# mavmap/mavmap

Hardware: AMD Instinct MI355X
Metric: global-BA LM iterations/sec (higher is better)
Workload: dtype f64; 1 GPU; C3: 500 images / 200000 points / 2000000 obs global BA, PINHOLE+OPENCV, 2 shared cameras; images=500, points=200000, observations=2000000, parallelism=single GPU, options=max_iter 200, ftol 1e-6, gtol 1e-10, ptol 1e-8, Cauchy a=1, refine intrinsics

## Files before the change

__graft_entry__.py:

```python
import os
import subprocess
import sys

ROOT = os.path.dirname(os.path.abspath(__file__))
if ROOT not in sys.path:
    sys.path.insert(0, ROOT)


REFERENCE_FM_SHIM_DEPS = (("tests", "shim", "shim_driver.cpp"), ("tests", "shim", "mock_mavba.cpp"), ("shim", "base3d", "bundle_adjustment.cc"),
                          ("shim", "base3d", "bundle_adjustment.h"), ("include", "mavba.h"))


def build() -> None:
    from mavmap_amd import build as b
    lib = b.build()
    assert os.path.exists(lib), lib
    subprocess.check_call(["make", "-C", os.path.join(ROOT, "oracle"), "-s"])
    subprocess.check_call(["make", "-C", os.path.join(ROOT, "oracle"), "-s", "-B", "ref"])
    ref_shim = os.path.join(ROOT, "oracle", "_ref", "_shim_mock_reffm.so")
    if os.path.exists(ref_shim):
        with open(ref_shim + ".sha256", "w") as fh:
            fh.write(b.files_digest(os.path.join(ROOT, *f) for f in REFERENCE_FM_SHIM_DEPS))
    host_src = os.path.join(ROOT, "tests", "host", "ba_math_host.cpp")
    host_so = os.path.join(ROOT, "tests", "host", "_ba_math_host.so")
    subprocess.check_call(["g++", "-O2", "-std=c++17", "-fPIC", "-shared", "-o", host_so, host_src])
    tri_src = os.path.join(ROOT, "tests", "host", "tri_math_host.cpp")
    tri_so = os.path.join(ROOT, "tests", "host", "_tri_math_host.so")
    subprocess.check_call(["g++", "-O2", "-std=c++17", "-fPIC", "-shared", "-o", tri_so, tri_src])
    p3p_src = os.path.join(ROOT, "tests", "host", "p3p_math_host.cpp")
    p3p_so = os.path.join(ROOT, "tests", "host", "_p3p_math_host.so")
    subprocess.check_call(["g++", "-O2", "-std=c++17", "-fPIC", "-shared", "-o", p3p_so, p3p_src])
    e5_src = os.path.join(ROOT, "tests", "host", "e5_math_host.cpp")
    e5_so = os.path.join(ROOT, "tests", "host", "_e5_math_host.so")
    subprocess.check_call(["g++", "-O2", "-std=c++17", "-fPIC", "-shared", "-o", e5_so, e5_src])
    import mavmap_amd
    L = mavmap_amd.load()
    from mavmap_amd import api
    for sym in api.EXPORTED_SYMBOLS + api.TRIANGULATE_SYMBOLS + api.ABSPOSE_SYMBOLS + api.RELPOSE_SYMBOLS + api.BACKSUB_TILES_SYMBOLS:
        getattr(L, sym)


def smoke() -> None:
    import mavmap_amd
    from mavmap_amd import synth
    from tests import oracle_lib

    if mavmap_amd.device_count() < 1:
        raise RuntimeError("smoke(): no HIP device visible — the mavba backend has no CPU path")
    p = synth.make_config("C3", scale=0.01, seed=7)
    opts = dict(max_num_iterations=200, function_tolerance=1e-6, gradient_tolerance=1e-10)
    pg, po = p.copy(), p.copy()
    cost, res = mavmap_amd.bundle_adjustment(pg, opts)
    oracle_lib.set_threads(1)
    ro, _ = oracle_lib.solve(po, oracle_lib.options(**opts))
    from tests.conftest import param_errors
    rel = abs(res["final_cost"] - ro["final_cost"]) / ro["final_cost"]
    errs = param_errors(pg, po)
    print(f"smoke: {p.num_images} images / {p.num_points} points / {p.num_obs} obs; "
          f"iterations {res['num_successful_steps'] + res['num_unsuccessful_steps']}; RMSE {cost:.6f} px; "
          f"vs oracle: cost {rel:.2e}, " + ", ".join(f"{k} {v:.1e}" for k, v in errs.items()))
    assert res["final_cost"] < res["initial_cost"]
    assert rel < 1e-6 and all(v < 1e-6 for v in errs.values()), (rel, errs)


if __name__ == "__main__":
    build()
    if "--smoke" in sys.argv:
        smoke()
```

mavmap_amd/api.py:

```python
import ctypes as C
import os
from dataclasses import dataclass

import numpy as np

from . import _abi as A
from .problem import BAProblem

_LIB_PATH = os.path.join(os.path.dirname(os.path.abspath(__file__)), "lib", "libmavba.so")
_lib = None

EXPORTED_SYMBOLS = [
    "mavba_options_init", "mavba_last_error", "mavba_device_count", "mavba_solve", "mavba_pose_refine",
    "mavba_session_create", "mavba_session_destroy", "mavba_session_reset", "mavba_session_iterate",
    "mavba_session_result", "mavba_session_get_params", "mavba_session_point_errors",
    "mavba_session_set_allreduce", "mavba_session_eval_jacobian", "mavba_session_reduced_dim",
    "mavba_session_reduced_system", "mavba_session_linear_step", "mavba_session_time_jacobian", "mavba_session_time_front", "mavba_session_set_profiling",
    "mavba_session_kernel_stats", "mavba_session_get_info", "mavba_dense_spd_solve",
    "mavba_scene_create", "mavba_scene_destroy", "mavba_scene_set_camera", "mavba_scene_set_image", "mavba_scene_add_point2d",
    "mavba_scene_add_points2d", "mavba_scene_set_point3d", "mavba_scene_link", "mavba_scene_delete_point3d", "mavba_scene_get_image", "mavba_scene_get_point3d",
    "mavba_scene_get_camera", "mavba_scene_flatten", "mavba_scene_bundle_adjust",
    "mavba_rccl_unique_id", "mavba_session_set_rccl", "mavba_pose_refine_batch", "mavba_session_set_params", "mavba_session_restart", "mavba_session_filter_points", "mavba_solve_filter_solve",
    "mavba_debug_elimination_tree", "mavba_debug_radix_sort", "mavba_debug_lm_decide", "mavba_debug_chol_schedule",
    "mavba_debug_inproc_comms", "mavba_debug_upload_batch",
]
TRIANGULATE_SYMBOLS = ["mavba_triangulate_pairs"]
ABSPOSE_SYMBOLS = ["mavba_absolute_pose_ransac"]
RELPOSE_SYMBOLS = ["mavba_relative_pose_ransac"]
BACKSUB_TILES_SYMBOLS = ["mavba_debug_backsub_tiles"]

ALLREDUCE_FN = C.CFUNCTYPE(C.c_int, C.c_void_p, C.c_void_p, C.c_int64, C.c_int32)


class MavbaError(RuntimeError):
    def __init__(self, code, msg):
        super().__init__(f"mavba error {code}: {msg}")
        self.code = code


def lib_path():
    return _LIB_PATH


def load():
    global _lib
    if _lib is not None:
        return _lib
    if not os.path.exists(_LIB_PATH):
        raise MavbaError(A.ERR_NO_DEVICE, f"{_LIB_PATH} is missing: run `python -m mavmap_amd.build` "
                                          "(the HIP extension is mandatory, there is no CPU fallback)")
    L = C.CDLL(_LIB_PATH)
    dp, ip, bp = C.POINTER(C.c_double), C.POINTER(C.c_int32), C.POINTER(C.c_uint8)
    pp, op, rp = C.POINTER(A.CProblem), C.POINTER(A.COptions), C.POINTER(A.CResult)
    sp = C.c_void_p
    L.mavba_options_init.argtypes = [op]
    L.mavba_options_init.restype = None
    L.mavba_last_error.restype = C.c_char_p
    L.mavba_device_count.restype = C.c_int
    L.mavba_solve.argtypes = [pp, op, rp, dp]
    L.mavba_pose_refine.argtypes = [dp, dp, dp, C.c_int32, dp, dp, bp, C.c_int64, op, rp]
    L.mavba_session_create.argtypes = [pp, op, C.POINTER(sp)]
    L.mavba_session_destroy.argtypes = [sp]
    L.mavba_session_destroy.restype = None
    L.mavba_session_reset.argtypes = [sp]
    L.mavba_session_iterate.argtypes = [sp, C.c_int32, ip, ip]
    L.mavba_session_result.argtypes = [sp, rp]
    L.mavba_session_get_params.argtypes = [sp, dp, dp, dp]
    L.mavba_session_point_errors.argtypes = [sp, dp]
    L.mavba_session_set_allreduce.argtypes = [sp, ALLREDUCE_FN, C.c_void_p, C.c_int32, C.c_int32]
    L.mavba_session_eval_jacobian.argtypes = [sp, dp, dp, dp, dp, dp]
    L.mavba_session_reduced_dim.argtypes = [sp]
    L.mavba_session_reduced_system.argtypes = [sp, C.c_double, dp, dp]
    L.mavba_session_linear_step.argtypes = [sp, C.c_double, dp, dp, dp, dp]
    L.mavba_session_time_jacobian.argtypes = [sp, C.c_int32, C.POINTER(C.c_float)]
    L.mavba_session_time_front.argtypes = [sp, C.c_double, C.c_int32, C.POINTER(C.c_float)]
    L.mavba_session_set_profiling.argtypes = [sp, C.c_int32]
    L.mavba_session_kernel_stats.argtypes = [sp, C.POINTER(A.CKernelStat), C.c_int32]
    L.mavba_session_get_info.argtypes = [sp, C.POINTER(A.CSessionInfo)]
    L.mavba_dense_spd_solve.argtypes = [C.c_int32, dp, dp, dp, C.c_int32]
    i64p, i64 = C.POINTER(C.c_int64), C.c_int64
    sop = C.POINTER(A.CSceneOptions)
    L.mavba_scene_create.argtypes = [C.POINTER(sp)]
    L.mavba_scene_destroy.argtypes = [sp]
    L.mavba_scene_destroy.restype = None
    L.mavba_scene_set_camera.argtypes = [sp, i64, C.c_int32, dp]
    L.mavba_scene_set_image.argtypes = [sp, i64, i64, dp, dp]
    L.mavba_scene_add_point2d.argtypes = [sp, i64, i64, dp]
    L.mavba_scene_add_points2d.argtypes = [sp, i64, i64, i64p, dp, i64p]
    L.mavba_scene_set_point3d.argtypes = [sp, i64, dp]
    L.mavba_scene_link.argtypes = [sp, i64, i64]
    L.mavba_scene_delete_point3d.argtypes = [sp, i64]
    L.mavba_scene_get_image.argtypes = [sp, i64, dp, dp]
    L.mavba_scene_get_point3d.argtypes = [sp, i64, dp]
    L.mavba_scene_get_camera.argtypes = [sp, i64, ip, dp]
    lists = [i64p, i64, i64p, i64, i64p, i64, i64p, i64, i64p, dp, i64]
    L.mavba_scene_flatten.argtypes = [sp] + lists + [sop, pp, C.POINTER(i64p), C.POINTER(i64p), C.POINTER(i64p)]
    L.mavba_scene_bundle_adjust.argtypes = [sp] + lists + [sop, op, rp, dp, C.POINTER(i64p), C.POINTER(dp), i64p]
    L.mavba_rccl_unique_id.argtypes = [C.c_void_p]
    L.mavba_session_set_rccl.argtypes = [sp, C.c_void_p, C.c_int32, C.c_int32]
    L.mavba_pose_refine_batch.argtypes = [C.c_int32, C.POINTER(A.CPoseRefineItem), op, rp]
    L.mavba_triangulate_pairs.argtypes = [C.c_int32, C.POINTER(A.CTriPair), C.c_int32]
    L.mavba_triangulate_pairs.restype = C.c_int
    L.mavba_absolute_pose_ransac.argtypes = [C.c_int32, C.POINTER(A.CAbsPoseItem), C.c_int32]
    L.mavba_absolute_pose_ransac.restype = C.c_int
    L.mavba_relative_pose_ransac.argtypes = [C.c_int32, C.POINTER(A.CRelPoseItem), C.c_int32]
    L.mavba_relative_pose_ransac.restype = C.c_int
    L.mavba_session_set_params.argtypes = [sp, dp, dp, dp]
    L.mavba_session_restart.argtypes = [sp]
    L.mavba_session_filter_points.argtypes = [sp, C.c_double, bp, bp, dp, C.POINTER(C.c_int64)]
    L.mavba_solve_filter_solve.argtypes = [pp, op, C.c_double, bp, rp, rp, dp, bp, C.POINTER(C.c_int64)]
    L.mavba_debug_elimination_tree.argtypes = [C.c_int32, C.c_int32, C.c_int64, ip, ip, C.c_int32, ip, ip, C.c_int32]
    L.mavba_debug_radix_sort.argtypes = [C.c_int32, C.POINTER(C.c_uint32), C.c_int32, ip, C.c_int32]
    L.mavba_debug_lm_decide.argtypes = [C.c_int32, dp, dp, dp, C.c_int32]
    L.mavba_debug_backsub_tiles.argtypes = [C.c_int32, ip, ip, C.c_int32]
    L.mavba_debug_backsub_tiles.restype = C.c_int
    i32p, i64p = C.POINTER(C.c_int32), C.POINTER(C.c_int64)
    L.mavba_debug_chol_schedule.argtypes = [C.c_int32, C.c_int32, i32p, i32p, i32p, C.c_int64, i32p, i32p, C.c_int32, dp,
                                            i32p, C.c_int64, i64p, i32p, C.c_int64, i64p, i32p]
    for f in EXPORTED_SYMBOLS:
        if f not in ("mavba_options_init", "mavba_last_error", "mavba_session_destroy", "mavba_scene_destroy", "mavba_debug_upload_batch"):
            getattr(L, f).restype = C.c_int
    _lib = L
    return L


def _check(rc):
    if rc != A.OK:
        raise MavbaError(rc, load().mavba_last_error().decode(errors="replace"))


def device_count():
    return int(load().mavba_device_count())


def _d(a):
    return A.ptr(a, C.c_double)


@dataclass
class BundleAdjustmentOptions:
    max_num_iterations: int = 100
    function_tolerance: float = 1e-4
    gradient_tolerance: float = 1e-8
    update_point3D_errors: bool = False
    min_track_len: int = 2
    loss_scale_factor: float = 1.0
    constrain_rotation: bool = False
    constrain_rotation_weight: float = 0.0
    refine_camera_params: bool = False
    print_progress: bool = False
    print_summary: bool = True

    @staticmethod
    def global_ba():
# ... 467 lines not shown
        self.close()

    def reset(self):
        _check(load().mavba_session_reset(self._h))

    def iterate(self, max_iters=1):
        done, term = C.c_int32(), C.c_int32()
        _check(load().mavba_session_iterate(self._h, int(max_iters), C.byref(done), C.byref(term)))
        return done.value, term.value

    def solve(self):
        self.iterate(self.copt.max_num_iterations + 1)
        return self.result()

    def result(self):
        r = A.CResult()
        _check(load().mavba_session_result(self._h, C.byref(r)))
        return r.as_dict()

    def get_params(self):
        p = self.problem
        poses, intr, pts = np.zeros((p.num_images, 6)), np.zeros((p.num_cameras, 9)), np.zeros((p.num_points, 3))
        _check(load().mavba_session_get_params(self._h, _d(poses), _d(intr), _d(pts)))
        return poses, intr, pts

    def point_errors(self):
        e = np.full(self.problem.num_points, np.nan)
        _check(load().mavba_session_point_errors(self._h, _d(e)))
        return e

    def set_params(self, poses=None, intrinsics=None, points=None):
        p = self.problem
        arrs = [None if a is None else A.as_f64(a, shape) for a, shape in
                ((poses, (p.num_images, 6)), (intrinsics, (p.num_cameras, 9)), (points, (p.num_points, 3)))]
        _check(load().mavba_session_set_params(self._h, *[None if a is None else _d(a) for a in arrs]))

    def restart(self):
        _check(load().mavba_session_restart(self._h))

    def filter_points(self, max_error, keep=None):
        n = self.problem.num_points
        removed, errors = np.zeros(n, np.uint8), np.full(n, np.nan)
        keep_arr = None if keep is None else np.ascontiguousarray(keep, dtype=np.uint8)
        cnt = C.c_int64()
        _check(load().mavba_session_filter_points(self._h, float(max_error), A.ptr(keep_arr, C.c_uint8),
                                                  A.ptr(removed, C.c_uint8), _d(errors), C.byref(cnt)))
        return removed, errors

    def set_allreduce(self, fn, rank, world_size):
        def trampoline(_ctx, ptr, count, op):
            try:
                fn(ptr, count, op)
                return 0
            except Exception as e:
                print("all-reduce hook raised:", repr(e), flush=True)
                return 1
        self._cb = ALLREDUCE_FN(trampoline)
        _check(load().mavba_session_set_allreduce(self._h, self._cb, None, rank, world_size))

    def set_rccl(self, unique_id, rank, world_size):
        buf = C.create_string_buffer(bytes(unique_id), 128)
        _check(load().mavba_session_set_rccl(self._h, buf, rank, world_size))

    def eval_jacobian(self):
        n = self.problem.num_obs
        r, Jc, Jp, Jk = np.zeros((n, 2)), np.zeros((n, 2, 6)), np.zeros((n, 2, 3)), np.zeros((n, 2, 9))
        cost = C.c_double()
        _check(load().mavba_session_eval_jacobian(self._h, C.byref(cost), _d(r), _d(Jc), _d(Jp), _d(Jk)))
        return cost.value, r, Jc, Jp, Jk

    def reduced_system(self, radius):
        n = load().mavba_session_reduced_dim(self._h)
        S, v = np.zeros((n, n)), np.zeros(n)
        _check(load().mavba_session_reduced_system(self._h, float(radius), _d(S), _d(v)))
        return S, v

    def linear_step(self, radius):
        p = self.problem
        dp, di, dx = np.zeros((p.num_images, 6)), np.zeros((p.num_cameras, 9)), np.zeros((p.num_points, 3))
        mcc = C.c_double()
        _check(load().mavba_session_linear_step(self._h, float(radius), _d(dp), _d(di), _d(dx), C.byref(mcc)))
        return dict(d_poses=dp, d_intr=di, d_points=dx, model_cost_change=mcc.value)

    def set_profiling(self, on):
        _check(load().mavba_session_set_profiling(self._h, 1 if on else 0))

    def time_front(self, radius=1e4, reps=20):
        ms = C.c_float(0)
        _check(load().mavba_session_time_front(self._h, float(radius), int(reps), C.byref(ms)))
        return ms.value

    def time_jacobian(self, reps=20):
        ms = C.c_float()
        _check(load().mavba_session_time_jacobian(self._h, int(reps), C.byref(ms)))
        return float(ms.value)

    def info(self):
        i = A.CSessionInfo()
        _check(load().mavba_session_get_info(self._h, C.byref(i)))
        d = {k: getattr(i, k) for k, _ in i._fields_ if k != "schur_terms"}
        d["schur_terms"] = list(i.schur_terms)
        return d

    def kernel_stats(self):
        buf = (A.CKernelStat * 64)()
        n = load().mavba_session_kernel_stats(self._h, buf, 64)
        return {buf[i].name.decode(): dict(launches=int(buf[i].launches), total_ms=float(buf[i].total_ms))
                for i in range(min(n, 64))}


def elimination_tree(num_images, num_cameras, pairs, max_depth=3):
    pairs = np.ascontiguousarray(pairs, dtype=np.int32).reshape(-1, 2)
    a, b = np.ascontiguousarray(pairs[:, 0]), np.ascontiguousarray(pairs[:, 1])
    node = np.zeros(max(num_images, 1), np.int32)
    parent = np.zeros(4096, np.int32)
    n = load().mavba_debug_elimination_tree(int(num_images), int(num_cameras), len(a), A.ptr(a, C.c_int32), A.ptr(b, C.c_int32),
                                           int(max_depth), A.ptr(node, C.c_int32), A.ptr(parent, C.c_int32), len(parent))
    if n < 0:
        _check(n)
    return node[:num_images], parent[:n]


def backsub_tiles(pt_start):
    pt_start = np.ascontiguousarray(pt_start, dtype=np.int32)
    num_points = max(len(pt_start) - 1, 0)
    out = np.zeros((max(num_points, 1), 4), np.int32)
    n = load().mavba_debug_backsub_tiles(num_points, A.ptr(pt_start, C.c_int32), A.ptr(out, C.c_int32), num_points)
    if n < 0:
        _check(n)
    return out[:n].copy()


def radix_sort_order(keys, key_bytes=4, device=-1):
    keys = np.ascontiguousarray(keys, dtype=np.uint32)
    out = np.zeros(len(keys), np.int32)
    _check(load().mavba_debug_radix_sort(len(keys), A.ptr(keys, C.c_uint32), int(key_bytes), A.ptr(out, C.c_int32), device))
    return out


def debug_upload_batch(sizes, arena_bytes=0, device=-1):
    sizes = np.ascontiguousarray(sizes, dtype=np.int64)
    f = load().mavba_debug_upload_batch
    f.restype = C.c_int64
    r = f(C.c_int32(len(sizes)), A.ptr(sizes, C.c_int64), C.c_int64(int(arena_bytes)), C.c_int32(device))
    if r < 0:
        raise MavbaError(A.ERR_HIP, load().mavba_last_error().decode(errors="replace"))
    return int(r)


def debug_lm_decide(cases, device=-1):
    cases = np.ascontiguousarray(cases, dtype=np.float64)
    n = cases.shape[0]
    assert cases.shape[1] == 24
    oh, od = np.zeros((n, 6)), np.zeros((n, 6))
    _check(load().mavba_debug_lm_decide(n, _d(cases), _d(oh), _d(od), device))
    return oh, od


def debug_chol_schedule(nb, nodes, pairs, cus=256):
    nodes = np.ascontiguousarray(nodes, dtype=np.int32).reshape(-1, 3)
    pairs = np.ascontiguousarray(pairs, dtype=np.int32).reshape(-1, 2)
    nbg, ne, npar = (np.ascontiguousarray(nodes[:, k]) for k in range(3))
    pr, pc = np.ascontiguousarray(pairs[:, 0]), np.ascontiguousarray(pairs[:, 1])
    i32 = lambda a: a.ctypes.data_as(C.POINTER(C.c_int32))
    out = np.zeros(8)
    nt, nu = C.c_int64(), C.c_int64()
# ... 25 lines not shown
```

mavmap_amd/build.py:

```python
import os
import shutil
import subprocess
import sys

ROOT = os.path.dirname(os.path.abspath(__file__))
CSRC = os.path.join(ROOT, "csrc")
LIBDIR = os.path.join(ROOT, "lib")
LIB = os.path.join(LIBDIR, "libmavba.so")
OBJDIR = os.path.join(LIBDIR, "obj")
SOURCES = ["kernels.hip", "schur_rows.hip", "dense_chol.hip", "pose_refine.hip", "triangulate.hip", "absolute_pose.hip", "relative_pose.hip", "host_util.hip", "session_build.hip", "session_lm.hip", "scene.hip", "multi_gpu.hip", "device_setup.hip", "api.hip"]
HEADERS = ["ba_math.h", "tri_math.h", "p3p_math.h", "e5_math.h", "dev_reduce.h", "internal.h", "session.h", "lm_decide.h", "lm_bodies.h", "sweep_body.h", "launch_dispatch.h", os.path.join("..", "..", "include", "mavba.h"),
           os.path.join("..", "..", "include", "mavba_triangulate.h"), os.path.join("..", "..", "include", "mavba_absolute_pose.h"),
           os.path.join("..", "..", "include", "mavba_relative_pose.h"), os.path.join("..", "..", "include", "mavba_backsub_tiles.h")]
FLAGS = ["--offload-arch=gfx950", "-O3", "-std=c++17", "-fPIC", "-ffp-contract=on", "-Wall",
         "-Wno-unused-result"]
FILE_FLAGS = {"dense_chol.hip": ["-mllvm", "-amdgpu-mfma-vgpr-form=1"]}


def _hipcc():
    for cand in (shutil.which("hipcc"), "/opt/rocm/bin/hipcc"):
        if cand and os.path.exists(cand):
            return cand
    raise RuntimeError("hipcc not found (ROCm toolchain required to build libmavba.so)")


STAMP = os.path.join(LIBDIR, "build_stamp.json")


def files_digest(paths):
    import hashlib
    h = hashlib.sha256()
    for p in paths:
        with open(p, "rb") as fh:
            h.update(os.path.basename(p).encode() + b"\0" + fh.read())
    return h.hexdigest()


def source_digest():
    import hashlib
    h = hashlib.sha256()
    for f in SOURCES + HEADERS:
        with open(os.path.normpath(os.path.join(CSRC, f)), "rb") as fh:
            h.update(f.encode() + b"\0" + fh.read())
    h.update(" ".join(FLAGS).encode())
    h.update(repr(sorted(FILE_FLAGS.items())).encode())
    return h.hexdigest()


def is_current():
    import json
    try:
        return os.path.exists(LIB) and json.load(open(STAMP))["digest"] == source_digest()
    except (OSError, ValueError, KeyError):
        return False


def _stale(target, deps):
    if not os.path.exists(target):
        return True
    t = os.path.getmtime(target)
    return any(os.path.getmtime(d) > t for d in deps if os.path.exists(d))


def build(force=False, verbose=False):
    if not force and is_current():
        return LIB
    os.makedirs(OBJDIR, exist_ok=True)
    hdrs = [os.path.normpath(os.path.join(CSRC, h)) for h in HEADERS]
    hipcc = _hipcc()
    objs = []
    for src in SOURCES:
        sp = os.path.join(CSRC, src)
        obj = os.path.join(OBJDIR, src.replace(".hip", ".o"))
        if force or _stale(obj, [sp] + hdrs):
            cmd = [hipcc] + FLAGS + FILE_FLAGS.get(src, []) + ["-c", sp, "-o", obj]
            if verbose:
                print(" ".join(cmd), file=sys.stderr)
            subprocess.check_call(cmd)
        objs.append(obj)
    if force or _stale(LIB, objs):
        cmd = [hipcc, "--offload-arch=gfx950", "-shared", "-fPIC", "-o", LIB] + objs
        if verbose:
            print(" ".join(cmd), file=sys.stderr)
        subprocess.check_call(cmd)
    if not is_current():
        import json
        with open(STAMP, "w") as fh:
            json.dump(dict(digest=source_digest()), fh)
    return LIB


if __name__ == "__main__":
    print(build(force="--force" in sys.argv, verbose=True))
```

mavmap_amd/csrc/api.hip:

```cpp
#include "session.h"
#include "lm_decide.h"

namespace mavba { thread_local std::string g_last_error; }

using namespace mavba;


#define MAVBA_TRY try {
namespace {
struct DeviceGuard {
  int prev = -1;
  explicit DeviceGuard(int dev) {
    if (hipGetDevice(&prev) != hipSuccess) { (void)hipGetLastError(); prev = -1; }
    if (prev != dev) HIP_OK(hipSetDevice(dev)); else prev = -1;
  }
  ~DeviceGuard() { if (prev >= 0) (void)hipSetDevice(prev); }
  DeviceGuard(const DeviceGuard&) = delete;
  DeviceGuard& operator=(const DeviceGuard&) = delete;
};
}
#define MAVBA_SESSION_TRY(s)                                                    \
  try {                                                                         \
    if (!(s)) throw Failure(MAVBA_ERR_INVALID_ARGUMENT, "null session");        \
    DeviceGuard device_guard_((s)->device);
// ... 302 lines not shown

int mavba_debug_backsub_tiles(int32_t NP, const int32_t* pt_start, int32_t* tiles_out, int32_t cap) {
  MAVBA_TRY
  if (NP < 0 || !pt_start || cap < 0 || (cap > 0 && !tiles_out)) throw Failure(MAVBA_ERR_INVALID_ARGUMENT, "bad argument");
  for (int q = 0; q < NP; ++q)
    if (pt_start[q + 1] < pt_start[q]) throw Failure(MAVBA_ERR_BAD_INDEX, "pt_start must not decrease");
  const std::vector<BsTile> tiles = build_backsub_tiles(pt_start, NP);
  if ((long long)tiles.size() > cap) throw Failure(MAVBA_ERR_INVALID_ARGUMENT, "tiles_out too small");
  for (size_t t = 0; t < tiles.size(); ++t) {
    tiles_out[4 * t] = tiles[t].p0; tiles_out[4 * t + 1] = tiles[t].np; tiles_out[4 * t + 2] = tiles[t].o0; tiles_out[4 * t + 3] = tiles[t].no;
  }
  return (int)tiles.size();
  MAVBA_CATCH
}

int mavba_debug_elimination_tree(int32_t NI, int32_t NC, int64_t npairs, const int32_t* pair_a, const int32_t* pair_b, int32_t max_depth,
                                 int32_t* node_of_image, int32_t* node_parent, int32_t cap) {
  MAVBA_TRY
  if (NI < 0 || NC < 0 || npairs < 0 || (npairs > 0 && (!pair_a || !pair_b)) || !node_of_image || !node_parent)
    throw Failure(MAVBA_ERR_INVALID_ARGUMENT, "bad argument");
  std::vector<std::vector<int>> lower(NI);
  for (int64_t k = 0; k < npairs; ++k) {
    const int a = pair_a[k], b = pair_b[k];
    if (a < 0 || a >= NI || b < 0 || b >= NI) throw Failure(MAVBA_ERR_BAD_INDEX, "image pair out of range");
    if (a != b) lower[std::max(a, b)].push_back(std::min(a, b));
  }
  const std::vector<ElimNode> tn = elimination_tree(NI, NC, lower, -1, max_depth);
  if ((int)tn.size() > cap) throw Failure(MAVBA_ERR_INVALID_ARGUMENT, "node_parent too small");
  for (int i = 0; i < NI; ++i) node_of_image[i] = -1;
  for (size_t t = 0; t < tn.size(); ++t) {
    node_parent[t] = tn[t].parent;
    for (int i : tn[t].imgs) node_of_image[i] = (int)t;
  }
  return (int)tn.size();
  MAVBA_CATCH
}

int mavba_session_reduced_system(mavba_session* s, double radius, double* Sout, double* vout) {
  MAVBA_SESSION_TRY(s)
  if (!s->evaluated) s->evaluate();
  s->assemble(radius);
  const int n = s->n_full, m = s->n_mat, nbt = m / 64;
  std::vector<double> store(s->chol_struct.store_doubles());
  s->download(store.data(), s->d_M.p, store.size() * 8);
  s->sync();
  std::vector<double> h((size_t)(m + 1) * m, 0.0);
  const std::vector<int>& slot = s->chol_struct.tile_slot;
  for (int tr = 0; tr <= nbt; ++tr)
    for (int tc = 0; tc < nbt; ++tc) {
      const int sl = slot[(size_t)tr * nbt + tc];
      if (sl < 0) continue;
      const double* T = &store[(size_t)sl << 12];
      const int rows = tr < nbt ? 64 : 1;
      for (int r = 0; r < rows; ++r) std::memcpy(&h[(size_t)(64 * tr + r) * m + 64 * tc], T + 64 * r, 64 * 8);
    }
  std::vector<int> var_col(n, 0);
  for (int t = 0; t < m; ++t) if (s->h_col_var[t] >= 0) var_col[s->h_col_var[t]] = t;
  if (Sout)
    for (int r = 0; r < n; ++r)
      for (int c = 0; c < n; ++c) {
        const int a = std::max(var_col[r], var_col[c]), b = std::min(var_col[r], var_col[c]);
        Sout[(size_t)r * n + c] = h[(size_t)a * m + b];
      }
  if (vout)
    for (int r = 0; r < n; ++r) vout[r] = h[(size_t)m * m + var_col[r]];
  return MAVBA_OK;
  MAVBA_CATCH
}

int mavba_session_linear_step(mavba_session* s, double radius, double* d_poses, double* d_intr, double* d_points,
                              double* model_cost_change) {
  MAVBA_SESSION_TRY(s)
  if (!s->evaluated) s->evaluate();
  double h[SC_COUNT];
  s->linear_step(radius, h);
  if (model_cost_change) *model_cost_change = h[SC_MODEL_CHANGE];
  if (d_poses && s->NI) s->download(d_poses, s->d_delta_cam.p, (size_t)s->NI * 48);
  if (d_intr && s->NC) s->download(d_intr, s->d_delta_cam.p + 6 * (size_t)s->NI, (size_t)s->NC * 72);
  std::vector<double> hdp;
  if (d_points && s->NP) { hdp.resize((size_t)s->NP * 3); s->download(hdp.data(), s->d_delta_pts.p, (size_t)s->NP * 24); }
  s->sync();
  if (d_points) s->to_caller_points(hdp.data(), d_points, 3);
  if (h[SC_FAIL] != 0.0 || h[SC_FAIL_FRONT] != 0.0) throw Failure(MAVBA_ERR_INVALID_ARGUMENT, "linear solve failed (matrix not positive definite)");
  return MAVBA_OK;
  MAVBA_CATCH
}

int mavba_session_time_jacobian(mavba_session* s, int32_t reps, float* ms_avg) {
  MAVBA_SESSION_TRY(s)
  if (reps < 1) reps = 1;
  s->ensure_planes();
  launch_cam_prepare(s->st, s->NI, s->d_poses.p, s->d_camrec.p);
  SweepArgs a = s->sweep_args(s->d_camrec.p, s->d_intr.p, s->d_points.p);
  for (int i = 0; i < 200; ++i) launch_jacobian_sweep(s->st, a);
  std::vector<hipEvent_t> ev((size_t)reps + 1);
  for (auto& e : ev) HIP_OK(hipEventCreate(&e));
  HIP_OK(hipEventRecord(ev[0], s->st));
  for (int i = 0; i < reps; ++i) {
    launch_jacobian_sweep(s->st, a);
    HIP_OK(hipEventRecord(ev[(size_t)i + 1], s->st));
  }
  HIP_OK(hipStreamSynchronize(s->st));
  float ms = 0.f;
  for (int i = 0; i < reps; ++i) {
    float one = 0.f;
    HIP_OK(hipEventElapsedTime(&one, ev[(size_t)i], ev[(size_t)i + 1]));
    ms += one;
  }
  for (auto& e : ev) (void)hipEventDestroy(e);
  if (ms_avg) *ms_avg = ms / reps;
  s->sync();
  return MAVBA_OK;
  MAVBA_CATCH
}

int mavba_debug_chol_schedule(int32_t nb, int32_t num_nodes, const int32_t* node_begin, const int32_t* node_end, const int32_t* node_parent,
                              int64_t num_pairs, const int32_t* pair_row, const int32_t* pair_col, int32_t cus, double* out,
                              int32_t* tasks_out, int64_t tasks_cap, int64_t* num_tasks, int32_t* upd_out, int64_t upd_cap,
                              int64_t* num_upd, int32_t* chain_info_out) {
  MAVBA_TRY
  if (nb < 1 || num_nodes < 0 || num_pairs < 0 || !out || !num_tasks || !num_upd || cus < 2) throw Failure(MAVBA_ERR_INVALID_ARGUMENT, "bad argument");
  std::vector<CholNode> tree;
  for (int n = 0; n < num_nodes; ++n) tree.push_back(CholNode{node_begin[n], node_end[n], node_parent[n]});
  std::vector<std::pair<int, int>> pairs;
  for (int64_t q = 0; q < num_pairs; ++q) {
    if (pair_row[q] < 0 || pair_row[q] >= nb || pair_col[q] < 0 || pair_col[q] > pair_row[q]) throw Failure(MAVBA_ERR_BAD_INDEX, "tile pair out of range");
    pairs.emplace_back(pair_row[q], pair_col[q]);
  }
  CholStructure cs;
  cs.host_only = true;
  cs.host_only_cus = cus;
  if (cs.build(nb, pairs, tree, nullptr) != hipSuccess) throw Failure(MAVBA_ERR_HIP, "structure build failed");
  out[0] = cs.persist_ok ? 1.0 : 0.0; out[1] = cs.predicted_forward_us; out[2] = cs.lpp_estimate_us; out[3] = cs.persist_grid;
  out[4] = cs.persist_chain_wgs; out[5] = (double)cs.persist_tiles; out[6] = (double)cs.persist_updates; out[7] = cs.nseg;
  *num_tasks = (int64_t)cs.h_tasks.size();
  *num_upd = (int64_t)cs.h_upd.size();
  if (tasks_out && (int64_t)cs.h_tasks.size() <= tasks_cap) {
    int wg = 0;
    for (size_t t = 0; t < cs.h_tasks.size(); ++t) {
      while (wg + 1 < (int)cs.h_wg_begin.size() && cs.h_wg_begin[wg + 1] <= (int)t) ++wg;
      const CholTask& T = cs.h_tasks[t];
      int32_t* o = tasks_out + 6 * t;
      o[0] = wg; o[1] = T.kind; o[2] = T.i; o[3] = T.j; o[4] = T.ub; o[5] = T.ue;
    }
  }
  if (upd_out && (int64_t)cs.h_upd.size() <= upd_cap) std::copy(cs.h_upd.begin(), cs.h_upd.end(), upd_out);
  if (chain_info_out) for (int j = 0; j < nb; ++j) chain_info_out[j] = j < (int)cs.h_chain_info.size() ? cs.h_chain_info[j] : 0;
  return MAVBA_OK;
  MAVBA_CATCH
}

int mavba_debug_lm_decide(int32_t n, const double* cases, double* out_host, double* out_device, int32_t device) {
  MAVBA_TRY
  if (n < 0 || (n > 0 && (!cases || !out_host || !out_device))) throw Failure(MAVBA_ERR_INVALID_ARGUMENT, "bad argument");
  for (int c = 0; c < n; ++c) {
    const double* q = cases + (size_t)c * (SC_COUNT + 8);
    LmSpec sp = lm_spec_off();
    sp.radius = q[SC_COUNT]; sp.decrease_factor = q[SC_COUNT + 1]; sp.ptol = q[SC_COUNT + 2]; sp.ftol = q[SC_COUNT + 3];
    sp.min_rel_dec = q[SC_COUNT + 4]; sp.max_radius = q[SC_COUNT + 5]; sp.abs_gtol = q[SC_COUNT + 6]; sp.pending_eval = q[SC_COUNT + 7] != 0.0;
    const LmDecision d = lm_decide(q, sp);
    double* o = out_host + (size_t)c * 6;
    o[0] = (double)d.code; o[1] = d.radius; o[2] = d.decrease_factor; o[3] = d.rel; o[4] = d.step_norm; o[5] = d.cost_change;
  }
  int ndev = 0;
  if (hipGetDeviceCount(&ndev) != hipSuccess || ndev <= 0) { (void)hipGetLastError(); throw Failure(MAVBA_ERR_NO_DEVICE, "no HIP device: the mavba backend has no CPU path"); }
  if (n == 0) return MAVBA_OK;
// ... 365 lines not shown
```

mavmap_amd/csrc/internal.h:

```cpp
#ifndef MAVBA_INTERNAL_H_
#define MAVBA_INTERNAL_H_

#include <hip/hip_runtime.h>
#include <stdint.h>

#include <utility>
#include <vector>
#include <functional>

namespace mavba {

constexpr int kPoseRec = 24;
constexpr int kIntrRec = 36;

constexpr int kImgRec = 81;
constexpr int kCamRec = 54;
constexpr int kSweepAcc = 135;

struct SweepChunk { int image; int begin; int end; };

enum { BLK_PP = 0, BLK_IP = 1, BLK_II = 2 };

struct SchurBlock {
  int kind;
// ... 46 lines not shown
constexpr unsigned rows_emit_entry(int src, int o, int tab_index) { return (unsigned)src | (unsigned)o << 13 | (unsigned)tab_index << 20; }
constexpr int kRowsListsCam = kClImagesMax, kRowsListsCams = 2 * kClImagesMax, kRowsLists = 2 * kClImagesMax + kClCamsMax + 1;
constexpr int kRowsPassSplit = 96;
#if defined(__HIPCC__)
__host__ __device__
#endif
inline int rows_class_of_rows(int rows) { return rows <= 16 * kRowsClassNT[0] ? 0 : rows <= 16 * kRowsClassNT[1] ? 1 : 2; }
#if defined(__HIPCC__)
__host__ __device__
#endif
inline int rows_count(int ni, int cam_rows) { return 6 * ni + cam_rows + 1; }

enum {
  SC_COST = 0,
  SC_XNORM2,
  SC_GRAD_MAX,
  SC_NEW_COST,
  SC_STEP_NORM2,
  SC_MODEL_CHANGE,
  SC_CAND_XNORM2,
  SC_FAIL,
  SC_FAIL_FRONT,
  SC_CAND_END,
  SC_EVAL_COUNT = SC_GRAD_MAX + 1,
  SC_CAND_BEGIN = SC_NEW_COST,
  SC_CAND_COUNT = SC_CAND_END - SC_CAND_BEGIN,
  SC_COUNT = 16
};

enum { LM_REJECTED = 0, LM_ACCEPTED = 1, LM_INVALID = 2, LM_TERM_PTOL = 3, LM_TERM_FTOL = 4, LM_TERM_GTOL = 5 };
struct LmSpec {
  const double* dec;
  const double* scal;
  double radius, decrease_factor;
  double ptol, ftol, min_rel_dec, max_radius, abs_gtol;
  int pending_eval;
};
struct LmDecision {
  int code;
  double radius, decrease_factor;
  double rel, step_norm, cost_change;
};
#if defined(__HIPCC__)
__host__ __device__
#endif
inline LmSpec lm_spec_off() { LmSpec s{}; s.dec = nullptr; s.scal = nullptr; return s; }

struct SweepArgs {
  int N, Nstride, NI, NC, KMAX;
  const double2* uv; const int* obs_img; const int* obs_pt;
  const double* camrec; const double* intr; const int* img_cam; const int* cam_model;
  const double* points;
  const unsigned char* pt_active;
  double loss_b, loss_inv_b;
  double* R; double* Jp; double* Jc; double* Jk;
  double* cost_partial;
};
int jacobian_sweep_grid(int N);
void launch_cam_prepare(hipStream_t st, int NI, const double* poses, double* camrec);
void launch_jacobian_sweep(hipStream_t st, const SweepArgs& a);
void launch_cost_only(hipStream_t st, const SweepArgs& a);
void launch_raw_residual_norm(hipStream_t st, const SweepArgs& a, double* out_norm);

void launch_point_reduce(hipStream_t st, int NP, int NPs, int Nstride, int KMAX, const int* pt_start,
                         const int* q_start, const int* q_cam, const int* obs_img, const int* img_cam,
                         const double* R, const double* Jp, const double* Jk, double* Cu, double* gu,
                         double* Wk );

constexpr int kFrontObs = 256, kFrontPts = 64, kFrontQ = 96, kFrontMaxGrid = 65536;
struct FrontTile { int p0, p1, o0, o1, q0, q1; };
struct FrontArgs {
  SweepArgs sw;
  int num_tiles, NPs;
  const FrontTile* tiles;
  const int* pt_start; const int* q_start; const int* q_cam; const int* q_pt;
  const unsigned char* pt_free;
  const double* scale_cam; const double* scale_pt;
  double radius, dmin, dmax;
  double* Cu; double* gu; double* Gi; double* h;
  double* Epose; double* Eintr;
  double* fail;
  long long* trace;
  LmSpec spec;
};
int point_front_grid(int num_tiles);
void launch_point_front(hipStream_t st, const FrontArgs& a, int kmax_intr, bool entries);

struct CamSweepArgs {
  int NI, NC;
  const SweepChunk* chunks; int num_chunks;
  const double2* im_uv; const int* im_pt;
  const double* camrec; const double* intr; const int* img_cam; const int* cam_model;
  const double* points; const unsigned char* pt_active; double loss_b, loss_inv_b;
  double* partial;
  LmSpec spec;
};
void launch_camera_sweep(hipStream_t st, const CamSweepArgs& a, int kmax, bool any_intr_free);
void launch_rot_prior(hipStream_t st, int n, const int* prior_img, const double* prior_R0, double w,
                      const double* poses, double* res, double* jac, double* cost_partial, const LmSpec& spec = lm_spec_off());

void launch_scales(hipStream_t st, int NI, int NC, int NP, int NPs, int jacobi,
                   const unsigned char* pose_free, const unsigned char* intr_free,
                   const unsigned char* pt_free, const double* img_rec, const double* cam_rec,
                   const double* Cu, double* scale_cam, double* scale_pt);

constexpr int kStateNormsCamBlocks = 64;

void launch_factor_entries_pose(hipStream_t st, int N, int Nstride, int NPs, const int* obs_img, const int* obs_pt,
                                const unsigned char* pt_free, const double* Jc, const double* Jp, const double* scale_cam,
                                const double* scale_pt, double* Gi, double* h, double* Epose, const int* pt_start,
                                const double* Cu, const double* gu, double radius, double dmin, double dmax, double* fail);
void launch_entries_intr(hipStream_t st, int Q, int NI, int NPs, const int* q_pt, const int* q_cam,
                         const double* Wk, const double* scale_cam, const double* scale_pt,
                         const double* Gi, const double* h, double* Eintr);

void launch_schur_chunks(hipStream_t st, int kind, int num_chunks, const SchurChunk* chunks,
                         const int2* terms, const double* Epose, const double* Eintr,
                         double* partial);
#if defined(__HIPCC__)
__host__ __device__
#endif
constexpr int schur_partial_stride(int kind) { return kind == BLK_PP ? 42 : kind == BLK_IP ? 54 : 90; }
void launch_schur_rows(hipStream_t st, const FrontArgs& a, int kmax_intr, bool generic, int num_clusters,
                       const SchurRowsCluster* clusters, const int* tab, const int* cl_lists, const unsigned short* obs_meta,
                       const unsigned long long* lanemap, const unsigned* emit_map, double* part_pp, double* part_ip, double* part_ii,
                       const struct CamSweepArgs* with_sweep = nullptr );
void rows_emit_map(int ni, int nc, int flags, std::vector<unsigned>& pass0, std::vector<unsigned>& pass1);
constexpr unsigned long long kRowsLanesIdentity = 0xFEDCBA9876543210ull;
void launch_schur_clusters(hipStream_t st, int num_clusters, const SchurCluster* clusters, const int* tab,
                           const int* pt_start, const int* q_start, const unsigned short* obs_meta,
                           const unsigned short* q_meta, const unsigned char* pt_clustered, const double* Epose,
                           const double* Eintr, const double* h, int NPs, double* part_pp, double* part_ip,
                           double* part_ii);
void launch_schur_finalize(hipStream_t st, int num_blocks, const SchurBlock* blocks,
                           const double* part_pp, const double* part_ip, const double* part_ii,
                           int NI, int NC, const int* slot, int nb, bool add_base, double radius, double dmin,
                           double dmax, const int* img_cam, const double* img_rec,
                           const double* cam_rec, const double* scale_cam, const int* off_img, const int* off_cam,
                           double* S);
void launch_tiles_copy(hipStream_t st, int num_tiles, const int* tiles, const int* slot, int nb, double* M, double* buf, bool to_buf);
void launch_fix_diag(hipStream_t st, int n_mat, const int* slot, bool add_one, const int* col_var,
                     const double* scale_cam, double* S);

int backsub_points_grid(int NP);
void launch_backsub_points_jvp(hipStream_t st, int NP, int NPs, int NI, double radius, double dmin, double dmax,
                               const SweepArgs& a, const int* pt_start, const double* delta_cam,
                               const unsigned char* pt_free, const double* Gi, const double* h, const double* Cu,
                               const double* gu, const double* scale_pt, double* cand_points, double* delta_points,
                               double* partial , const double* cand_camrec = nullptr, const double* cand_intr = nullptr,
                               double* cost_partial = nullptr);
struct BsTile { int p0, np, o0, no; };
constexpr int kBsTileObs = 64, kBsTilePts = 64;
std::vector<BsTile> build_backsub_tiles(const int* pt_start, int NP);
int backsub_tiles_grid(int num_tiles);
void launch_backsub_points_tiles(hipStream_t st, int num_tiles, const BsTile* tiles, int NPs, int NI, double radius, double dmin,
                                 double dmax, const SweepArgs& a, const int* pt_start, const double* delta_cam,
                                 const unsigned char* pt_free, const double* Gi, const double* h, const double* Cu,
                                 const double* gu, const double* scale_pt, double* cand_points, double* delta_points,
                                 double* partial , const double* cand_camrec, const double* cand_intr,
                                 double* cost_partial);
struct CamUpdateArgs {
  int NI, NC, cam_part; double radius, dmin, dmax;
  const double* scale_cam; const double* img_rec; const double* cam_rec; const double* poses; const double* intr;
  double* cand_poses; double* cand_intr; double* delta_cam; double* partial3 ; double* cand_camrec;
};
int update_cameras_groups(int NI);
void launch_update_cameras(hipStream_t st, const CamUpdateArgs& u, const double* y);

struct ReduceTask { const double* src; int rows, stride, is_max; const double* src2; int rows2; double* out; };
struct ReduceTasks { ReduceTask t[6]; };
void launch_reduce_tasks(hipStream_t st, const ReduceTasks& tasks, int n, const LmSpec& spec = lm_spec_off());
constexpr int kLmPubDoubles = SC_COUNT + 8;
void launch_lm_snapshot(hipStream_t st, const LmSpec& spec, double* dec, double* host_pub, double seq, double* fail_slots );
void launch_lm_decide_cases(hipStream_t st, int n, const double* in, double* out);
void launch_lm_tail(hipStream_t st, const ReduceTasks& tasks, int n, const LmSpec& spec, double* dec, double* host_pub, double seq, double* fail_slots);
void state_norms_grid(int NI, int NC, int NP, int* gp, int* gc);
struct EvalTailArgs {
  int NI, NC, NP, NPs, with_cams, cam_part, gp, gc, num_tasks;
  int first_group = 0;
  const int* img_chunk_start; const double* cam_partial; const int* prior_start; const double* prior_res; const double* prior_jac;
  const int* cam_img_start; const int* cam_imgs; double* img_rec; double* cam_rec; double* img_intr_tmp;
  const unsigned char* pose_free; const unsigned char* intr_free; const unsigned char* pt_free;
  const double* poses; const double* intr; const double* points; const double* gu; double* norm_partial;
  ReduceTasks T; LmSpec spec;
  PartialRide ride;
};
void launch_camera_reduce(hipStream_t st, const EvalTailArgs& a);
void launch_state_norms(hipStream_t st, const EvalTailArgs& a);
void launch_eval_small(hipStream_t st, const EvalTailArgs& a);
void launch_eval_head_tail(hipStream_t st, const EvalTailArgs& a);

void launch_points_to_caller(hipStream_t st, int NP, int width, const int* orig, const double* in, double* out);
void launch_point_errors(hipStream_t st, int NP, const int* pt_start, const double* rnorm,
                         const int* pt_count, double* perr);

hipError_t device_alloc(void** p, size_t bytes);
void device_free(void* p);
hipError_t copy_h2d_staged(void* dst, const void* src, size_t bytes, hipStream_t st);
hipError_t copy_d2h_staged_sync(void* dst, const void* src, size_t bytes, hipStream_t st);
void release_staged(hipStream_t st);
bool upload_batch_begin(hipStream_t st);
hipError_t upload_batch_end(bool emit);
hipError_t zero_async(void* p, size_t bytes, hipStream_t st);
void upload_batch_debug_arena(size_t bytes);
int host_threads();
void host_run(int T, const std::function<void(int)>& body);

struct CholFront {
  int k;
  int na;
  int act_off;
  int factor_next;
  int sh_begin;
  long long sh_off;
};
struct CholStep { int kind, front_off, nf, nf0, max_na, merge_begin, init_off, tasks; };
struct CholMerge { int sh_begin; long long sh_off; };
struct CholNode { int begin, end, parent; };
enum { CHOL_TASK_TILE = 0, CHOL_TASK_PRE_DIAG = 1, CHOL_TASK_PRE_SUB = 2, CHOL_TASK_CHAIN = 3 };
struct CholTask { int kind, i, j, ub, ue; };
struct CholStructure {
  int nb = 0, nseg = 1;
// ... 63 lines not shown
```

mavmap_amd/csrc/kernels.hip:

```cpp
#include "internal.h"
#include <cstdlib>
#include <type_traits>
#include "ba_math.h"
#include "dev_reduce.h"
#include "lm_decide.h"
#include "lm_bodies.h"
#include "sweep_body.h"
#include "launch_dispatch.h"

namespace mavba {

__global__ void k_cam_prepare(int NI, const double* __restrict__ poses, double* __restrict__ camrec) {
  const int i = blockIdx.x * blockDim.x + threadIdx.x;
  if (i >= NI) return;
  double rec[9];
  cam_prepare(poses + 6 * i, rec);
#pragma unroll
  for (int k = 0; k < 9; ++k) camrec[9 * i + k] = rec[k];
}
void launch_cam_prepare(hipStream_t st, int NI, const double* poses, double* camrec) {
  if (NI <= 0) return;
  hipLaunchKernelGGL(k_cam_prepare, dim3((NI + 127) / 128), dim3(128), 0, st, NI, poses, camrec);
}

// ... 630 lines not shown
}

template <int K>
__global__ void __launch_bounds__(256, 2) k_camera_sweep_gram(CamSweepArgs a) {
  if (!lm_spec_go(a.spec, nullptr)) return;
  __shared__ __attribute__((aligned(16))) double s_rows[kCsLdsDoubles];
  camera_sweep_gram_body<K>(a, blockIdx.x, s_rows);
}
void launch_camera_sweep(hipStream_t st, const CamSweepArgs& a, int kmax, bool any_intr_free) {
  if (a.num_chunks <= 0) return;
  const dim3 g(a.num_chunks), b(256);
  if (!any_intr_free) hipLaunchKernelGGL(k_camera_sweep, g, b, 0, st, a);
  else with_width(kmax, [&](auto k) { hipLaunchKernelGGL((k_camera_sweep_gram<decltype(k)::value>), g, b, 0, st, a); });
}

__global__ void k_rot_prior(int n, const int* __restrict__ prior_img, const double* __restrict__ R0,
                            double w, const double* __restrict__ poses, double* __restrict__ res,
                            double* __restrict__ jac, double* __restrict__ cost_partial, LmSpec spec) {
  if (!lm_spec_go(spec, nullptr)) return;
  const int q = blockIdx.x * blockDim.x + threadIdx.x;
  if (q >= n) return;
  double r, j[3];
  rot_prior_eval(poses + 6 * prior_img[q], R0 + 9 * q, w, r, j);
  res[q] = r; jac[3 * q] = j[0]; jac[3 * q + 1] = j[1]; jac[3 * q + 2] = j[2];
  cost_partial[q] = 0.5 * r * r;
}
void launch_rot_prior(hipStream_t st, int n, const int* prior_img, const double* prior_R0, double w,
                      const double* poses, double* res, double* jac, double* cost_partial, const LmSpec& spec) {
  if (n <= 0) return;
  hipLaunchKernelGGL(k_rot_prior, dim3((n + 127) / 128), dim3(128), 0, st, n, prior_img, prior_R0, w, poses, res, jac, cost_partial, spec);
}

__device__ void partial_reduce_task(const PartialReduce T, int lane, double* part_pp, double* part_ip, double* part_ii);
__global__ void __launch_bounds__(64) k_camera_reduce_img(
    int NI, const int* __restrict__ img_chunk_start, const double* __restrict__ partial,
    const int* __restrict__ prior_start, const double* __restrict__ prior_res,
    const double* __restrict__ prior_jac, double* __restrict__ img_rec, double* __restrict__ img_intr_tmp, LmSpec spec, PartialRide ride) {
  if (!lm_spec_go(spec, nullptr)) return;
  if ((int)blockIdx.x >= NI) { partial_reduce_task(ride.tasks[blockIdx.x - NI], threadIdx.x, ride.pp, ride.ip, ride.ii); return; }
  camera_reduce_img_body(blockIdx.x, threadIdx.x, img_chunk_start, partial, prior_start, prior_res, prior_jac, img_rec, img_intr_tmp);
}
__global__ void __launch_bounds__(1024) k_camera_reduce_cam(
    const int* __restrict__ cam_img_start, const int* __restrict__ cam_imgs,
    const double* __restrict__ img_intr_tmp, double* __restrict__ cam_rec, LmSpec spec) {
  __shared__ double s_part[16][64];
  if (!lm_spec_go(spec, nullptr)) return;
  const int c = blockIdx.x;
  const int e = threadIdx.x & 63, part = threadIdx.x >> 6;
  double s = 0.0;
  if (e < kCamRec) {
    const int t1 = cam_img_start[c + 1];
    for (int t = cam_img_start[c] + part; t < t1; t += 64) {
      const int i0 = cam_imgs[t], i1 = cam_imgs[min(t + 16, t1 - 1)], i2 = cam_imgs[min(t + 32, t1 - 1)], i3 = cam_imgs[min(t + 48, t1 - 1)];
      const double x0 = img_intr_tmp[(size_t)i0 * kCamRec + e], x1 = img_intr_tmp[(size_t)i1 * kCamRec + e];
      const double x2 = img_intr_tmp[(size_t)i2 * kCamRec + e], x3 = img_intr_tmp[(size_t)i3 * kCamRec + e];
      s += x0;
      if (t + 16 < t1) s += x1;
      if (t + 32 < t1) s += x2;
      if (t + 48 < t1) s += x3;
    }
  }
  s_part[part][e] = s;
  __syncthreads();
  if (part == 0 && e < kCamRec) {
    double tot = 0.0;
#pragma unroll
    for (int k = 0; k < 16; ++k) tot += s_part[k][e];
    cam_rec[(size_t)c * kCamRec + e] = tot;
  }
}
void launch_camera_reduce(hipStream_t st, const EvalTailArgs& a) {
  if (a.NI > 0 || a.ride.n > 0)
    hipLaunchKernelGGL(k_camera_reduce_img, dim3(a.NI + a.ride.n), dim3(64), 0, st, a.NI, a.img_chunk_start, a.cam_partial,
                       a.prior_start, a.prior_res, a.prior_jac, a.img_rec, a.img_intr_tmp, a.spec, a.ride);
  if (a.NC > 0 && a.with_cams)
    hipLaunchKernelGGL(k_camera_reduce_cam, dim3(a.NC), dim3(1024), 0, st, a.cam_img_start, a.cam_imgs, a.img_intr_tmp, a.cam_rec, a.spec);
}

__global__ void k_scales(int NI, int NC, int NP, int NPs, int jacobi,
                         const unsigned char* __restrict__ pose_free,
                         const unsigned char* __restrict__ intr_free,
                         const unsigned char* __restrict__ pt_free, const double* __restrict__ img_rec,
                         const double* __restrict__ cam_rec, const double* __restrict__ Cu,
                         double* __restrict__ scale_cam, double* __restrict__ scale_pt) {
  const int t = blockIdx.x * blockDim.x + threadIdx.x;
  const int ncam = 6 * NI + 9 * NC;
  if (t < ncam) {
    double n2; bool fr;
    if (t < 6 * NI) {
      const int i = t / 6, e = t % 6;
      n2 = img_rec[(size_t)i * kImgRec + sym_idx(e, e, 6)];
      fr = pose_free[t] != 0;
    } else {
      const int c = (t - 6 * NI) / 9, k = (t - 6 * NI) % 9;
      n2 = cam_rec[(size_t)c * kCamRec + sym_idx(k, k, 9)];
      fr = intr_free[9 * c + k] != 0;
    }
    scale_cam[t] = fr ? (jacobi ? 1.0 / (1.0 + sqrt(n2)) : 1.0) : 0.0;
  }
  if (t < NP) {
    const bool fr = pt_free[t] != 0;
    const int d[3] = {0, 3, 5};
#pragma unroll
    for (int k = 0; k < 3; ++k)
      scale_pt[k * NPs + t] = fr ? (jacobi ? 1.0 / (1.0 + sqrt(Cu[d[k] * NPs + t])) : 1.0) : 0.0;
  }
}
void launch_scales(hipStream_t st, int NI, int NC, int NP, int NPs, int jacobi,
                   const unsigned char* pose_free, const unsigned char* intr_free,
                   const unsigned char* pt_free, const double* img_rec, const double* cam_rec,
                   const double* Cu, double* scale_cam, double* scale_pt) {
  const int n = max(6 * NI + 9 * NC, NP);
  if (n <= 0) return;
  hipLaunchKernelGGL(k_scales, dim3((n + 255) / 256), dim3(256), 0, st, NI, NC, NP, NPs, jacobi, pose_free,
                     intr_free, pt_free, img_rec, cam_rec, Cu, scale_cam, scale_pt);
}

__global__ void __launch_bounds__(256) k_state_norms(
    int NI, int NC, int NP, int NPs, int gp, int cam_part, const unsigned char* __restrict__ pose_free,
    const unsigned char* __restrict__ intr_free, const unsigned char* __restrict__ pt_free,
    const double* __restrict__ poses, const double* __restrict__ intr, const double* __restrict__ points,
    const double* __restrict__ img_rec, const double* __restrict__ cam_rec, const double* __restrict__ gu,
    double* __restrict__ partial, LmSpec spec) {
  __shared__ double s_red[4];
  if (!lm_spec_go(spec, nullptr)) return;
  state_norms_body(blockIdx.x, gp, gridDim.x - gp, NI, NC, NP, NPs, cam_part, pose_free, intr_free, pt_free, poses, intr, points,
                   img_rec, cam_rec, gu, partial, s_red);
}
void state_norms_grid(int NI, int NC, int NP, int* gp, int* gc) {
  *gp = std::min(512, (NP + 255) / 256);
  *gc = std::max(1, std::min(kStateNormsCamBlocks, (6 * NI + 9 * NC + 255) / 256));
}
void launch_state_norms(hipStream_t st, const EvalTailArgs& a) {
  hipLaunchKernelGGL(k_state_norms, dim3(a.gp + a.gc), dim3(256), 0, st, a.NI, a.NC, a.NP, a.NPs, a.gp, a.cam_part, a.pose_free,
                     a.intr_free, a.pt_free, a.poses, a.intr, a.points, a.img_rec, a.cam_rec, a.gu, a.norm_partial, a.spec);
}


__global__ void __launch_bounds__(256) k_entries_pose(
    int N, int Nstride, int NPs, const int* __restrict__ obs_img, const int* __restrict__ obs_pt,
    const unsigned char* __restrict__ pt_free, const double* __restrict__ Jc, const double* __restrict__ Jp,
    const double* __restrict__ scale_cam, const double* __restrict__ scale_pt, double* __restrict__ Gi,
    double* __restrict__ h, double* __restrict__ Epose, const int* __restrict__ pt_start, const double* __restrict__ Cu,
    const double* __restrict__ gu, double radius, double dmin, double dmax, double* __restrict__ fail) {
  __shared__ double s_rec[256 * 25];
  const long long S = Nstride;
  const long long o = (long long)blockIdx.x * 256 + threadIdx.x;
  double rec[kPoseRec];
#pragma unroll
  for (int k = 0; k < kPoseRec; ++k) rec[k] = 0.0;
  if (o < N) {
    const int p = obs_pt[o];
    const bool fr = pt_free[p] != 0;
    if (!fr && o == pt_start[p]) {
#pragma unroll
      for (int k = 0; k < 6; ++k) Gi[k * NPs + p] = 0.0;
#pragma unroll
      for (int k = 0; k < 3; ++k) h[k * NPs + p] = 0.0;
    }
    if (fr) {
      const int im = obs_img[o];
      double sp[3], G[6], hh[3], jp[6];
#pragma unroll
      for (int k = 0; k < 3; ++k) sp[k] = scale_pt[k * NPs + p];
      double C[6];
      C[0] = sp[0] * sp[0] * Cu[p];           C[1] = sp[0] * sp[1] * Cu[NPs + p];     C[2] = sp[0] * sp[2] * Cu[2 * NPs + p];
      C[3] = sp[1] * sp[1] * Cu[3 * NPs + p]; C[4] = sp[1] * sp[2] * Cu[4 * NPs + p]; C[5] = sp[2] * sp[2] * Cu[5 * NPs + p];
      C[0] += clampd(C[0], dmin, dmax) / radius;
      C[3] += clampd(C[3], dmin, dmax) / radius;
      C[5] += clampd(C[5], dmin, dmax) / radius;
      const bool ok = chol3_inv(C, G);
      const double gs[3] = {sp[0] * gu[p], sp[1] * gu[NPs + p], sp[2] * gu[2 * NPs + p]};
      gi_mul(G, gs, hh);
      if (o == pt_start[p]) {
        bool fin = ok;
#pragma unroll
        for (int k = 0; k < 6; ++k) fin = fin && isfinite(G[k]);
        if (!fin) atomicAdd(fail, 1.0);
#pragma unroll
        for (int k = 0; k < 6; ++k) Gi[k * NPs + p] = G[k];
#pragma unroll
        for (int k = 0; k < 3; ++k) h[k * NPs + p] = hh[k];
      }
#pragma unroll
      for (int row = 0; row < 2; ++row)
#pragma unroll
        for (int k = 0; k < 3; ++k) jp[row * 3 + k] = Jp[(row * 3 + k) * S + o] * sp[k];
#pragma unroll
      for (int e = 0; e < 6; ++e) {
        const double sc = scale_cam[6 * im + e];
        const double j0 = Jc[e * S + o] * sc, j1 = Jc[(6 + e) * S + o] * sc;
        const double w0 = j0 * jp[0] + j1 * jp[3], w1 = j0 * jp[1] + j1 * jp[4], w2 = j0 * jp[2] + j1 * jp[5];
        const double u0 = w0 * G[0];
        const double u1 = w0 * G[1] + w1 * G[2];
        const double u2 = w0 * G[3] + w1 * G[4] + w2 * G[5];
        rec[3 * e] = u0; rec[3 * e + 1] = u1; rec[3 * e + 2] = u2;
        rec[18 + e] = u0 * hh[0] + u1 * hh[1] + u2 * hh[2];
      }
// ... 362 lines not shown
    switch (wv) {
      case 0: cluster_mfma<SH, 0>(E, lane, acc); break;
      case 1: cluster_mfma<SH, 1>(E, lane, acc); break;
      case 2: cluster_mfma<SH, 2>(E, lane, acc); break;
      case 3: cluster_mfma<SH, 3>(E, lane, acc); break;
      case 4: cluster_mfma<SH, 4>(E, lane, acc); break;
      case 5: cluster_mfma<SH, 5>(E, lane, acc); break;
      case 6: cluster_mfma<SH, 6>(E, lane, acc); break;
      default: cluster_mfma<SH, 7>(E, lane, acc); break;
    }
    __syncthreads();
  }
  const int* tab = s_tab;
  switch (wv) {
    case 0: cluster_emit<SH, 0>(lane, acc, tab, part_pp, part_ip, part_ii); break;
    case 1: cluster_emit<SH, 1>(lane, acc, tab, part_pp, part_ip, part_ii); break;
    case 2: cluster_emit<SH, 2>(lane, acc, tab, part_pp, part_ip, part_ii); break;
    case 3: cluster_emit<SH, 3>(lane, acc, tab, part_pp, part_ip, part_ii); break;
    case 4: cluster_emit<SH, 4>(lane, acc, tab, part_pp, part_ip, part_ii); break;
    case 5: cluster_emit<SH, 5>(lane, acc, tab, part_pp, part_ip, part_ii); break;
    case 6: cluster_emit<SH, 6>(lane, acc, tab, part_pp, part_ip, part_ii); break;
    default: cluster_emit<SH, 7>(lane, acc, tab, part_pp, part_ip, part_ii); break;
  }
}
void launch_schur_clusters(hipStream_t st, int num_clusters, const SchurCluster* clusters, const int* tab,
                           const int* pt_start, const int* q_start, const unsigned short* obs_meta,
                           const unsigned short* q_meta, const unsigned char* pt_clustered, const double* Epose,
                           const double* Eintr, const double* h, int NPs, double* part_pp, double* part_ip,
                           double* part_ii) {
  if (num_clusters <= 0) return;
  hipLaunchKernelGGL(k_schur_clusters, dim3(num_clusters), dim3(kClThreads), 0, st, clusters, tab, pt_start, q_start, obs_meta,
                     q_meta, pt_clustered, Epose, Eintr, h, NPs, part_pp, part_ip, part_ii);
}

void launch_schur_chunks(hipStream_t st, int kind, int num_chunks, const SchurChunk* chunks,
                         const int2* terms, const double* Epose, const double* Eintr, double* partial) {
  if (num_chunks <= 0) return;
  const dim3 g((((num_chunks + 3) / 4) + 7) / 8 * 8), b(256);
  if (kind == BLK_PP)
    hipLaunchKernelGGL((k_schur_chunks<6, 6, kPoseRec, kPoseRec, true>), g, b, 0, st, num_chunks, chunks, terms, Epose, Epose, partial);
  else if (kind == BLK_IP)
    hipLaunchKernelGGL((k_schur_chunks<9, 6, kIntrRec, kPoseRec, false>), g, b, 0, st, num_chunks, chunks, terms, Eintr, Epose, partial);
  else
    hipLaunchKernelGGL((k_schur_chunks<9, 9, kIntrRec, kIntrRec, true>), g, b, 0, st, num_chunks, chunks, terms, Eintr, Eintr, partial);
}

__device__ __forceinline__ double strided_sum16(const double* __restrict__ part, int PS, int idx, int begin, int end) {
  double s[16];
#pragma unroll
  for (int u = 0; u < 16; ++u) s[u] = 0.0;
  for (int c = begin; c < end; c += 16) {
    double x[16];
#pragma unroll
    for (int u = 0; u < 16; ++u) x[u] = part[(size_t)min(c + u, end - 1) * PS + idx];
#pragma unroll
    for (int u = 0; u < 16; ++u) s[u] += (c + u < end) ? x[u] : 0.0;
  }
  return (((s[0] + s[1]) + (s[2] + s[3])) + ((s[4] + s[5]) + (s[6] + s[7]))) + (((s[8] + s[9]) + (s[10] + s[11])) + ((s[12] + s[13]) + (s[14] + s[15])));
}
__device__ void partial_reduce_task(const PartialReduce T, int lane, double* part_pp, double* part_ip, double* part_ii) {
  double* part = T.kind == BLK_PP ? part_pp : T.kind == BLK_IP ? part_ip : part_ii;
  const int PS = schur_partial_stride(T.kind);
  for (int idx = lane; idx < PS; idx += 64) part[(size_t)T.dst * PS + idx] = strided_sum16(part, PS, idx, T.src_begin, T.src_end);
}
__global__ void __launch_bounds__(256) k_partial_reduce(int num_tasks, const PartialReduce* __restrict__ tasks,
                                                        double* __restrict__ part_pp, double* __restrict__ part_ip,
                                                        double* __restrict__ part_ii) {
  const int task = blockIdx.x * 4 + (threadIdx.x >> 6), lane = threadIdx.x & 63;
  if (task >= num_tasks) return;
  partial_reduce_task(tasks[task], lane, part_pp, part_ip, part_ii);
}
void launch_partial_reduce(hipStream_t st, int num_tasks, const PartialReduce* tasks, double* part_pp, double* part_ip,
                           double* part_ii) {
  if (num_tasks <= 0) return;
  hipLaunchKernelGGL(k_partial_reduce, dim3((num_tasks + 3) / 4), dim3(256), 0, st, num_tasks, tasks, part_pp, part_ip, part_ii);
}

__global__ void __launch_bounds__(256) k_schur_finalize(
    int num_blocks, const SchurBlock* __restrict__ blocks, const double* __restrict__ part_pp,
    const double* __restrict__ part_ip, const double* __restrict__ part_ii, int NI, int NC, const int* __restrict__ slot, int nb,
    int add_base, double radius, double dmin, double dmax, const int* __restrict__ img_cam,
    const double* __restrict__ img_rec, const double* __restrict__ cam_rec,
    const double* __restrict__ scale_cam, const int* __restrict__ off_img, const int* __restrict__ off_cam,
    double* __restrict__ S) {
  const int wv = threadIdx.x >> 6, lane = threadIdx.x & 63;
  const int bid = blockIdx.x * 4 + wv;
  if (bid >= num_blocks) return;
  const SchurBlock B = blocks[bid];
  const int RX = B.kind == BLK_PP ? 6 : 9, RY = B.kind == BLK_II ? 9 : 6;
  const int NA = RX * RY;
  const bool diag_kind = B.kind != BLK_IP;
  const int PS = NA + (diag_kind ? RX : 0);
  const double* part = B.kind == BLK_PP ? part_pp : B.kind == BLK_IP ? part_ip : part_ii;
  const int row0 = B.kind == BLK_PP ? 6 * B.row_ent : 6 * NI + 9 * B.row_ent;
  const int col0 = B.kind == BLK_II ? 6 * NI + 9 * B.col_ent : 6 * B.col_ent;
  const int prow0 = B.kind == BLK_PP ? off_img[B.row_ent] : off_cam[B.row_ent];
  const int pcol0 = B.kind == BLK_II ? off_cam[B.col_ent] : off_img[B.col_ent];
  const bool is_diag = diag_kind && B.row_ent == B.col_ent;
  auto apply = [&](int idx, double s) {
    if (idx < NA) {
      const int r = idx / RY, c = idx - r * RY;
      const int gr = row0 + r, gc = col0 + c;
      double base = 0.0;
      if (add_base) {
        const double sr = scale_cam[gr], sc = scale_cam[gc];
        if (B.kind == BLK_PP && is_diag) {
          const int x = r < c ? r : c, y = r < c ? c : r;
          base = sr * sc * img_rec[(size_t)B.row_ent * kImgRec + sym_idx(x, y, 6)];
          if (r == c && sr != 0.0) base += clampd(base, dmin, dmax) / radius;
        } else if (B.kind == BLK_IP && img_cam[B.col_ent] == B.row_ent) {
          base = sr * sc * img_rec[(size_t)B.col_ent * kImgRec + 27 + c * 9 + r];
        } else if (B.kind == BLK_II && is_diag) {
          const int x = r < c ? r : c, y = r < c ? c : r;
          base = sr * sc * cam_rec[(size_t)B.row_ent * kCamRec + sym_idx(x, y, 9)];
          if (r == c && sr != 0.0) base += clampd(base, dmin, dmax) / radius;
        }
      }
      double val = base - s;
      if (is_diag && r == c && scale_cam[gr] == 0.0) val = add_base ? 1.0 : 0.0;
      if (!is_diag || r >= c) {
        const int R = prow0 + r, C = pcol0 + c;
        if ((R >> 6) >= (C >> 6)) S[((size_t)slot[(R >> 6) * nb + (C >> 6)] << 12) + (R & 63) * 64 + (C & 63)] = val;
        if ((C >> 6) >= (R >> 6)) S[((size_t)slot[(C >> 6) * nb + (R >> 6)] << 12) + (C & 63) * 64 + (R & 63)] = val;
      }
    } else if (is_diag) {
      const int r = idx - NA;
      const int gr = row0 + r;
      double base = 0.0;
      if (add_base) {
        const double g = B.kind == BLK_PP ? img_rec[(size_t)B.row_ent * kImgRec + 21 + r]
                                          : cam_rec[(size_t)B.row_ent * kCamRec + 45 + r];
        base = scale_cam[gr] * g;
      }
      const int C = prow0 + r;
      S[((size_t)slot[nb * nb + (C >> 6)] << 12) + (C & 63)] = base - s;
    }
  };
  for (int idx = lane; idx < PS; idx += 64) apply(idx, strided_sum16(part, PS, idx, B.chunk_begin, B.chunk_end));
}
void launch_schur_finalize(hipStream_t st, int num_blocks, const SchurBlock* blocks,
                           const double* part_pp, const double* part_ip, const double* part_ii,
                           int NI, int NC, const int* slot, int nb, bool add_base, double radius, double dmin,
                           double dmax, const int* img_cam, const double* img_rec,
                           const double* cam_rec, const double* scale_cam, const int* off_img, const int* off_cam,
                           double* S) {
  if (num_blocks <= 0) return;
  hipLaunchKernelGGL(k_schur_finalize, dim3((num_blocks + 3) / 4), dim3(256), 0, st, num_blocks, blocks, part_pp,
                     part_ip, part_ii, NI, NC, slot, nb, add_base ? 1 : 0, radius, dmin, dmax, img_cam, img_rec, cam_rec,
                     scale_cam, off_img, off_cam, S);
}
__global__ void __launch_bounds__(256) k_tiles_copy(int num_tiles, const int* __restrict__ tiles, const int* __restrict__ slot, int nb,
                                                    double* __restrict__ M, double* __restrict__ buf, int to_buf) {
  const int t = blockIdx.x;
  if (t < num_tiles) {
    double2* a = reinterpret_cast<double2*>(M + ((size_t)tiles[t] << 12));
    double2* b = reinterpret_cast<double2*>(buf + ((size_t)t << 12));
    for (int e = threadIdx.x; e < 2048; e += 256) { if (to_buf) b[e] = a[e]; else a[e] = b[e]; }
  } else {
    double* rhs = buf + ((size_t)num_tiles << 12);
    for (int c = (t - num_tiles) * 256 + threadIdx.x; c < nb * 64; c += (gridDim.x - num_tiles) * 256) {
      double* a = M + ((size_t)slot[nb * nb + (c >> 6)] << 12) + (c & 63);
      if (to_buf) rhs[c] = *a; else *a = rhs[c];
    }
  }
}
void launch_tiles_copy(hipStream_t st, int num_tiles, const int* tiles, const int* slot, int nb, double* M, double* buf, bool to_buf) {
  const int extra = std::max(1, std::min(16, (nb * 64 + 1023) / 1024));
  hipLaunchKernelGGL(k_tiles_copy, dim3(num_tiles + extra), dim3(256), 0, st, num_tiles, tiles, slot, nb, M, buf, to_buf ? 1 : 0);
}

__global__ void k_fix_diag(int n_mat, const int* __restrict__ slot, int add_one, const int* __restrict__ col_var,
                           const double* __restrict__ scale_cam, double* __restrict__ S) {
  const int t = blockIdx.x * blockDim.x + threadIdx.x;
  if (t >= n_mat) return;
  const int j = col_var[t];
  if (j < 0 || scale_cam[j] == 0.0) S[((size_t)slot[(t >> 6) * (n_mat >> 6) + (t >> 6)] << 12) + (t & 63) * 65] = add_one ? 1.0 : 0.0;
}
void launch_fix_diag(hipStream_t st, int n_mat, const int* slot, bool add_one, const int* col_var, const double* scale_cam, double* S) {
  hipLaunchKernelGGL(k_fix_diag, dim3((n_mat + 255) / 256), dim3(256), 0, st, n_mat, slot, add_one ? 1 : 0, col_var, scale_cam, S);
}

constexpr int kBsCamsLds = 16;
__global__ void __launch_bounds__(256) k_backsub_points_packed(
    int NP, int NPs, int NI, int NC, int N, int ppb, int nblocks, double radius, double dmin, double dmax, double loss_b, double loss_inv_b,
    const int* __restrict__ pt_start, const int* __restrict__ obs_img, const int* __restrict__ obs_pt,
    const double2* __restrict__ uv, const int* __restrict__ img_cam, const int* __restrict__ cam_model,
    const double* __restrict__ camrec, const double* __restrict__ intr, const double* __restrict__ delta_cam,
    const unsigned char* __restrict__ pt_free, const double* __restrict__ Gi, const double* __restrict__ h,
    const double* __restrict__ Cu, const double* __restrict__ gu, const double* __restrict__ scale_pt,
    const double* __restrict__ points, double* __restrict__ cand_points, double* __restrict__ delta_points,
    double* __restrict__ partial, const double* __restrict__ cand_camrec, const double* __restrict__ cand_intr,
    const unsigned char* __restrict__ pt_active, double* __restrict__ cost_partial) {
  __shared__ double s_t[3][256];
  __shared__ double s_new[3][128];
  __shared__ double s_red[4];
  __shared__ double s_kin[kBsCamsLds][9], s_dk[kBsCamsLds][9];
  __shared__ int s_model[kBsCamsLds];
  const int tid = threadIdx.x;
  const bool cams_lds = NC <= kBsCamsLds;
  double a_step = 0.0, a_model = 0.0, a_x2 = 0.0, a_cost = 0.0;
  const int G = (int)gridDim.x;
  struct Obs { int pt, im; double2 m; };
  auto load_obs = [&](int o) {
    Obs r{0, 0, make_double2(0.0, 0.0)};
    if (N <= 0) return r;
    const int oc = min(o, N - 1);
    r.pt = obs_pt[oc]; r.im = obs_img[oc]; r.m = uv[oc];
    return r;
  };
  auto obs_term = [&](const Obs& q, bool valid, double (&t)[3]) {
    t[0] = t[1] = t[2] = 0.0;
    if (!valid || !pt_free[q.pt]) return;
    const int cam = img_cam[q.im];
    const double X[3] = {points[3 * (size_t)q.pt], points[3 * (size_t)q.pt + 1], points[3 * (size_t)q.pt + 2]};
    double rec[9], kin[9], dc[6], dk[9];
#pragma unroll
    for (int k = 0; k < 9; ++k) rec[k] = camrec[9 * q.im + k];
#pragma unroll
    for (int k = 0; k < 6; ++k) dc[k] = delta_cam[6 * q.im + k];
    int model;
    if (cams_lds) {
      model = s_model[cam];
#pragma unroll
      for (int k = 0; k < 9; ++k) { kin[k] = s_kin[cam][k]; dk[k] = s_dk[cam][k]; }
    } else {
      model = cam_model[cam];
#pragma unroll
      for (int k = 0; k < 9; ++k) { kin[k] = intr[9 * cam + k]; dk[k] = delta_cam[6 * NI + 9 * cam + k]; }
    }
    double r[2], tt[3];
#ifndef MAVBA_BS_SKIP
#define MAVBA_BS_SKIP 0
// ... 461 lines not shown
```

mavmap_amd/csrc/schur_rows.hip:

```cpp
#include "internal.h"
#include <cstdio>
#include <cstdlib>
#include <type_traits>
#include <vector>
#include "ba_math.h"
#include "dev_reduce.h"
#include "lm_decide.h"
#include "sweep_body.h"
#include "launch_dispatch.h"

#ifndef MAVBA_ROWS_SKIP
#define MAVBA_ROWS_SKIP 0
#endif

namespace mavba {
namespace {
typedef double f2_d4 __attribute__((ext_vector_type(4)));
constexpr int kF2Threads = 256, kF2Waves = 4;
constexpr int kF2K = 3 * kRowsBatch, kF2Pitch = kF2K + 2;
static_assert(kRowsBatch == 16, "one point per 16-lane DPP row");
static_assert((2 * kF2Pitch) % 8 == 4, "pitch must spread the 16 operand rows over all banks");
constexpr int kF2TabIP = kClTabIP, kF2TabII = kClTabII, kF2Tab = kClTab;

template <int CTRL>
// ... 54 lines not shown
      ++t;
    }
  return false;
}
template <int NT>
struct F2Shape { static constexpr int rows = 16 * NT, tiles = NT * (NT + 1) / 2, acc = (tiles + kF2Waves - 1) / kF2Waves; };
template <int NT, int W>
__device__ __forceinline__ void f2_mfma(const double* __restrict__ E, int lane, f2_d4 (&acc)[F2Shape<NT>::acc]) {
  const int li = lane & 15, lk = lane >> 4;
  const double* base = E + li * kF2Pitch + lk;
  auto load = [&](double (&x)[NT], int kk) {
#pragma unroll
    for (int i = 0; i < NT; ++i)
      if (f2_row_used<NT>(W, i)) x[i] = base[16 * i * kF2Pitch + kk];
  };
  auto mma = [&](const double (&x)[NT]) {
    int t = 0;
#pragma unroll
    for (int i = 0; i < NT; ++i)
#pragma unroll
      for (int j = 0; j <= i; ++j) {
        if (t % kF2Waves == W) acc[t / kF2Waves] = __builtin_amdgcn_mfma_f64_16x16x4f64(x[i], x[j], acc[t / kF2Waves], 0, 0, 0);
        ++t;
      }
  };
  static_assert(kF2K % 8 == 0, "two k-steps per trip");
  double a[NT], b[NT];
  load(a, 0);
#pragma unroll 1
  for (int kk = 0; kk < kF2K; kk += 8) {
    load(b, kk + 4);
    __builtin_amdgcn_sched_barrier(0);
    mma(a);
    __builtin_amdgcn_sched_barrier(0);
    if (kk + 8 < kF2K) load(a, kk + 8);
    __builtin_amdgcn_sched_barrier(0);
    mma(b);
    __builtin_amdgcn_sched_barrier(0);
  }
}
__host__ __device__ constexpr int f2_tri(int R) { return (R * (R + 1)) >> 1; }
template <int NT, int W, int RLO, int RHI>
__device__ __forceinline__ void f2_stage(double* __restrict__ T, int lane, const f2_d4 (&acc)[F2Shape<NT>::acc]) {
  const int li = lane & 15, lk = lane >> 4;
  const double* Tl = T + (f2_tri(lk) + li);
  int t = 0;
#pragma unroll
  for (int i = 0; i < NT; ++i)
#pragma unroll
    for (int j = 0; j <= i; ++j) {
      if (t % kF2Waves == W && 16 * i >= RLO && 16 * i < RHI) {
#pragma unroll
        for (int r = 0; r < 4; ++r) {
          const int R0 = 16 * i + 4 * r;
          double* dst = const_cast<double*>(Tl) + R0 * lk + (f2_tri(R0) - f2_tri(RLO) + 16 * j);
          if (i > j || li <= lk + 4 * r) *dst = acc[t / kF2Waves][r];
        }
      }
      ++t;
    }
}
__device__ __forceinline__ void f2_write_blocks(const double* __restrict__ T, int tid, const unsigned* __restrict__ map, int n,
                                                double* const* __restrict__ s_dst) {
  constexpr int U = 8;
  for (int e0 = tid; e0 < n; e0 += U * kF2Threads) {
    unsigned m[U];
#pragma unroll
    for (int u = 0; u < U; ++u) m[u] = e0 + u * kF2Threads < n ? map[e0 + u * kF2Threads] : 0u;
    double* d[U];
    double v[U];
#pragma unroll
    for (int u = 0; u < U; ++u) {
      d[u] = e0 + u * kF2Threads < n ? s_dst[m[u] >> 20] : nullptr;
      const unsigned src = m[u] & 8191u;
      v[u] = src == kRowsEmitZero ? 0.0 : T[src];
    }
#pragma unroll
    for (int u = 0; u < U; ++u) if (d[u]) d[u][(m[u] >> 13) & 127u] = v[u];
  }
}
}

struct RowsSweep { CamSweepArgs cs; int first; };
template <int KMAX, bool GENERIC, bool TRACE = false, bool SWEEP = false>
__global__ void __launch_bounds__(kF2Threads, 2) k_schur_rows(
    FrontArgs a, const SchurRowsCluster* __restrict__ clusters, const int* __restrict__ tabs, const int* __restrict__ cl_lists,
    const unsigned short* __restrict__ obs_meta, const unsigned long long* __restrict__ lanemap,
    const unsigned* __restrict__ emit_map, double* __restrict__ part_pp, double* __restrict__ part_ip, double* __restrict__ part_ii,
    RowsSweep sweep) {
  using SHMAX = F2Shape<kRowsClassNT[kRowsClasses - 1]>;
  if (!lm_spec_go(a.spec, &a.radius)) return;
  long long t_entry = 0, t_loop0 = 0, t_loop1 = 0;
  if constexpr (TRACE) t_entry = (long long)__builtin_amdgcn_s_memtime();
  __shared__ double s_rec[kClImagesMax][9], s_kin[kClImagesMax][9], s_sc[kClImagesMax][6], s_ksc[kClCamsMax][9];
  __shared__ int s_icam[kClImagesMax], s_model[kClImagesMax], s_lc[kClImagesMax], s_clcam[4];
  constexpr int kELen = (SWEEP && KMAX > 0 && kCsLdsDoubles > SHMAX::rows * kF2Pitch) ? kCsLdsDoubles : SHMAX::rows * kF2Pitch;
  __shared__ __attribute__((aligned(16))) double E[kELen];
  if constexpr (SWEEP) {
    static_assert(kF2Threads == 256 && SHMAX::rows * kF2Pitch >= 4 * kSweepAcc, "the sweep's chunk layout and scratch");
    if ((int)blockIdx.x >= sweep.first) {
      if constexpr (KMAX == 0) camera_sweep_body(sweep.cs, (int)blockIdx.x - sweep.first, E);
      else camera_sweep_gram_body<KMAX>(sweep.cs, (int)blockIdx.x - sweep.first, E);
      return;
    }
  }
  __shared__ double s_red[kF2Waves];
  __shared__ double* s_dst[kF2Tab];
  __shared__ int s_pstart[kRowsMaxPoints + 1];
  __shared__ unsigned long long s_lanes[kRowsMaxPoints];
  const int tid = threadIdx.x, wv = tid >> 6, lane = tid & 63, r = tid >> 4, i = tid & 15;
  const SweepArgs& w = a.sw;
  const int NPs = a.NPs;
  const int cidx = blockIdx.x;
  const SchurRowsCluster cl = clusters[cidx];
  const int npts = cl.p1 - cl.p0, nbatch = (npts + kRowsBatch - 1) / kRowsBatch;
  const int P0 = 6 * cl.ni, H = P0 + rows_cam_rows(cl.flags);
  for (int j = tid; j <= npts; j += kF2Threads) s_pstart[j] = a.pt_start[cl.p0 + j];
  for (int j = tid; j < npts; j += kF2Threads) s_lanes[j] = lanemap[cl.p0 + j];
  if (tid < kF2Tab) {
    const int slot = tabs[(size_t)cidx * kF2Tab + tid];
    s_dst[tid] = slot < 0 ? nullptr : tid < kF2TabIP ? part_pp + (size_t)slot * 42 : tid < kF2TabII ? part_ip + (size_t)slot * 54 : part_ii + (size_t)slot * 90;
  }
  {
    const int* lists = cl_lists + (size_t)cidx * kRowsLists;
    if (tid < kClImagesMax * 9) {
      const int sl = tid / 9, e = tid - 9 * sl, img = lists[sl];
      if (img >= 0) {
        const int cam = lists[kRowsListsCam + sl];
        s_rec[sl][e] = w.camrec[9 * img + e];
        s_kin[sl][e] = w.intr[9 * cam + e];
        if (e < 6) s_sc[sl][e] = a.scale_cam[6 * img + e];
        if (e == 0) {
          s_icam[sl] = cam; s_model[sl] = w.cam_model[cam];
          s_lc[sl] = cam == lists[kRowsListsCams] ? 0 : cam == lists[kRowsListsCams + 1] ? 1 : cam == lists[kRowsListsCams + 2] ? 2 : -1;
        }
      }
    } else if (tid < kClImagesMax * 9 + kClCamsMax * 9) {
      const int t = tid - kClImagesMax * 9, c = t / 9, k = t - 9 * c, cam = lists[kRowsListsCams + c];
      if (cam >= 0) s_ksc[c][k] = a.scale_cam[6 * w.NI + 9 * cam + k];
      if (k == 0) s_clcam[c] = cam;
    }
  }
  double cost = 0.0;
  auto run = [&](auto nt_const) {
  constexpr int NT = decltype(nt_const)::value;
  using SH = F2Shape<NT>;
  f2_d4 acc[SH::acc];
#pragma unroll
  for (int t = 0; t < SH::acc; ++t) acc[t] = (f2_d4){0.0, 0.0, 0.0, 0.0};
  long long stamp[TRACE ? 8 : 1];
  int nstamp = 0;
  bool tracing = false;
  auto mark = [&]() { if constexpr (TRACE) { if (tracing && nstamp < 8) stamp[nstamp++] = (long long)__builtin_amdgcn_s_memtime(); } };
  bool act_n = false, free_n = false, seen_n = false;
  int im_n = 0;
  double2 m_n = make_double2(0.0, 0.0);
  unsigned meta_n = 0xFFFFu;
  double X_n[3] = {0.0, 0.0, 0.0}, sp_n[3] = {0.0, 0.0, 0.0};
  auto request_point = [&](int pj, int ob, int cnt, unsigned long long lm) {
    const int p = cl.p0 + pj;
    const bool on = w.pt_active == nullptr || w.pt_active[p] != 0;
    const int oi = (int)(((i & 8) ? (unsigned)(lm >> 32) : (unsigned)lm) >> (4 * (i & 7))) & 15;
    seen_n = cnt > 0;
    act_n = on && oi < cnt;
    if (act_n) { im_n = w.obs_img[ob + oi]; m_n = w.uv[ob + oi]; meta_n = obs_meta[ob + oi]; }
    X_n[0] = w.points[3 * (size_t)p]; X_n[1] = w.points[3 * (size_t)p + 1]; X_n[2] = w.points[3 * (size_t)p + 2];
    free_n = a.pt_free[p] != 0;
#pragma unroll
    for (int k = 0; k < 3; ++k) sp_n[k] = a.scale_pt[(size_t)k * NPs + p];
  };
  auto request_batch = [&](int bj) {
    const int pj = bj * kRowsBatch + r;
    act_n = free_n = seen_n = false;
    if (pj < npts) { const int ob = s_pstart[pj]; request_point(pj, ob, s_pstart[pj + 1] - ob, s_lanes[pj]); }
  };
  if (r < npts) { const int ob = a.pt_start[cl.p0 + r]; request_point(r, ob, a.pt_start[cl.p0 + r + 1] - ob, lanemap[cl.p0 + r]); }
  __syncthreads();
  if constexpr (TRACE) t_loop0 = (long long)__builtin_amdgcn_s_memtime();
  for (int bi = 0; bi < nbatch; ++bi) {
    const int pj = bi * kRowsBatch + r;
    const bool valid = pj < npts, act = act_n, own_free = free_n, seen = seen_n;
    const int im = im_n;
    const double2 m = m_n;
    const unsigned meta = act ? meta_n : 0xFFFFu;
    const double X[3] = {X_n[0], X_n[1], X_n[2]};
    const double own_sp[3] = {sp_n[0], sp_n[1], sp_n[2]};
    if constexpr (TRACE) tracing = bi == 1;
    lds_barrier();
    mark();
    constexpr int K3 = KMAX > 0 ? 3 * KMAX : 1;
    const double sp[3] = {own_free ? own_sp[0] : 0.0, own_free ? own_sp[1] : 0.0, own_free ? own_sp[2] : 0.0};
    double jc[12], jps[6], s9[9], P[K3];
#pragma unroll
    for (int e = 0; e < 9; ++e) s9[e] = 0.0;
#pragma unroll
    for (int u = 0; u < K3; ++u) P[u] = 0.0;
    int mylc = -1;
    if (act) {
      int model, cam;
      double rec[9], kin[9];
      if (meta != 0xFFFFu) {
        const int sl = (int)(meta >> 8);
        cam = s_icam[sl];
        model = s_model[sl];
        mylc = s_lc[sl];
#pragma unroll
        for (int k = 0; k < 9; ++k) { rec[k] = s_rec[sl][k]; kin[k] = s_kin[sl][k]; }
      } else {
        cam = w.img_cam[im];
        model = w.cam_model[cam];
#pragma unroll
        for (int k = 0; k < 9; ++k) rec[k] = w.camrec[9 * im + k];
#pragma unroll
        for (int k = 0; k < 9; ++k) kin[k] = w.intr[9 * cam + k];
        if constexpr (KMAX > 0) mylc = cam == s_clcam[0] ? 0 : cam == s_clcam[1] ? 1 : cam == s_clcam[2] ? 2 : -1;
      }
      double res[2], Jc[12], Jp[6], Jk[18];
      double wgt, half_rho;
#if MAVBA_ROWS_SKIP & 4
      res[0] = m.x * rec[0] + kin[0]; res[1] = m.y * rec[1] + X[0];
      for (int e = 0; e < 12; ++e) Jc[e] = res[0] + e;
      for (int e = 0; e < 6; ++e) Jp[e] = res[1] + e;
      for (int e = 0; e < 18; ++e) Jk[e] = res[1] - e + model;
      wgt = 0.5; half_rho = res[0];
#else
      obs_jacobian(model, rec, kin, X, m.x, m.y, res, Jc, Jp, Jk);
      cauchy_weight(res[0] * res[0] + res[1] * res[1], w.loss_b, w.loss_inv_b, wgt, half_rho);
#endif
      cost += half_rho;
      const double rr0 = wgt * res[0], rr1 = wgt * res[1];
#pragma unroll
      for (int e = 0; e < 12; ++e) jc[e] = wgt * Jc[e];
      double jp[6];
#pragma unroll
      for (int e = 0; e < 6; ++e) jp[e] = wgt * Jp[e];
      s9[0] = jp[0] * jp[0] + jp[3] * jp[3]; s9[1] = jp[0] * jp[1] + jp[3] * jp[4]; s9[2] = jp[0] * jp[2] + jp[3] * jp[5];
      s9[3] = jp[1] * jp[1] + jp[4] * jp[4]; s9[4] = jp[1] * jp[2] + jp[4] * jp[5]; s9[5] = jp[2] * jp[2] + jp[5] * jp[5];
      s9[6] = jp[0] * rr0 + jp[3] * rr1; s9[7] = jp[1] * rr0 + jp[4] * rr1; s9[8] = jp[2] * rr0 + jp[5] * rr1;
#pragma unroll
      for (int e = 0; e < 6; ++e) jps[e] = jp[e] * sp[e % 3];
      const double wgt_k = (GENERIC || mylc >= 0) ? wgt : 0.0;
#pragma unroll
      for (int k = 0; k < KMAX; ++k) {
        const double k0 = wgt_k * Jk[k], k1 = wgt_k * Jk[9 + k];
#pragma unroll
        for (int t = 0; t < 3; ++t) P[3 * k + t] = k0 * jps[t] + k1 * jps[3 + t];
      }
    }
    mark();
#if !(MAVBA_ROWS_SKIP & 16)
    row16_allsum(s9);
#endif
    double G[6] = {0, 0, 0, 0, 0, 0}, hh[3] = {0, 0, 0};
    bool fin = true;
    if (own_free) {
      double C[6];
      C[0] = sp[0] * sp[0] * s9[0]; C[1] = sp[0] * sp[1] * s9[1]; C[2] = sp[0] * sp[2] * s9[2];
      C[3] = sp[1] * sp[1] * s9[3]; C[4] = sp[1] * sp[2] * s9[4]; C[5] = sp[2] * sp[2] * s9[5];
      const double inv_radius = 1.0 / a.radius;
      C[0] = __builtin_fma(clampd(C[0], a.dmin, a.dmax), inv_radius, C[0]);
      C[3] = __builtin_fma(clampd(C[3], a.dmin, a.dmax), inv_radius, C[3]);
      C[5] = __builtin_fma(clampd(C[5], a.dmin, a.dmax), inv_radius, C[5]);
#if MAVBA_ROWS_SKIP & 16
      for (int k = 0; k < 6; ++k) G[k] = C[k];
#else
      fin = chol3_inv_fast(C, G);
#endif
      const double gs[3] = {sp[0] * s9[6], sp[1] * s9[7], sp[2] * s9[8]};
      gi_mul(G, gs, hh);
#pragma unroll
      for (int k = 0; k < 6; ++k) fin = fin && isfinite(G[k]);
    }
    if (valid && i == 0) {
      const int p = cl.p0 + pj;
#pragma unroll
      for (int k = 0; k < 6; ++k) a.Cu[(size_t)k * NPs + p] = s9[k];
#pragma unroll
      for (int k = 0; k < 3; ++k) a.gu[(size_t)k * NPs + p] = s9[6 + k];
      if (seen) {
#pragma unroll
        for (int k = 0; k < 6; ++k) a.Gi[(size_t)k * NPs + p] = G[k];
#pragma unroll
        for (int k = 0; k < 3; ++k) a.h[(size_t)k * NPs + p] = hh[k];
      }
      if (!fin) atomicAdd(a.fail, 1.0);
    }
    mark();
    double* col = E + 3 * r;
#if !(MAVBA_ROWS_SKIP & 32)
#pragma unroll
    for (int rb = 0; rb < NT; ++rb) {
      double* e = col + (16 * rb + i) * kF2Pitch;
      e[0] = 0.0; e[1] = 0.0; e[2] = 0.0;
    }
#endif
    if (act && meta != 0xFFFFu && !(MAVBA_ROWS_SKIP & 8)) {
      double* Eo = col + 6 * (int)(meta >> 8) * kF2Pitch;
      const double* scl = s_sc[meta >> 8];
      const double m00 = jps[0] * G[0], m01 = jps[0] * G[1] + jps[1] * G[2], m02 = jps[0] * G[3] + jps[1] * G[4] + jps[2] * G[5];
      const double m10 = jps[3] * G[0], m11 = jps[3] * G[1] + jps[4] * G[2], m12 = jps[3] * G[3] + jps[4] * G[4] + jps[5] * G[5];
#pragma unroll
      for (int e = 0; e < 6; ++e) {
        const double sc = scl[e];
        const double j0 = jc[e] * sc, j1 = jc[6 + e] * sc;
        Eo[e * kF2Pitch] = j0 * m00 + j1 * m10;
        Eo[e * kF2Pitch + 1] = j0 * m01 + j1 * m11;
        Eo[e * kF2Pitch + 2] = j0 * m02 + j1 * m12;
      }
    }
    if (i < 3 && own_free && seen) col[H * kF2Pitch + i] = hh[i];
    if constexpr (KMAX > 0 && !(MAVBA_ROWS_SKIP & 2)) {
      auto write_row = [&](int lc, int k, const double* W) {
        const int r0 = rows_cam_off(cl.flags, lc);
        if (k >= rows_cam_off(cl.flags, lc + 1) - r0) return;
        const double sk = s_ksc[lc][k];
        const double w0 = W[0] * sk, w1 = W[1] * sk, w2 = W[2] * sk;
        double* Eo = col + (P0 + r0 + k) * kF2Pitch;
        Eo[0] = w0 * G[0];
        Eo[1] = w0 * G[1] + w1 * G[2];
        Eo[2] = w0 * G[3] + w1 * G[4] + w2 * G[5];
      };
      if constexpr (!GENERIC) {
        static_assert(KMAX == 8 || KMAX == 4, "the in-place form is written for 4 and 8 parameters");
        if (cl.nc < 2) {
#pragma unroll
          for (int u = 0; u < K3; ++u) P[u] += xlane_f64<kDppMirror>(P[u]);
        } else if (cl.flags & kRowsUnplaced) {
          const bool up1 = i >= 8;
          const bool keepm = mylc == (up1 ? 1 : 0), sendm = mylc == (up1 ? 0 : 1);
#pragma unroll
          for (int u = 0; u < K3; ++u) {
            const double keep = keepm ? P[u] : 0.0, send = sendm ? P[u] : 0.0;
            P[u] = keep + xlane_f64<kDppMirror>(send);
          }
        }
// ... 60 lines not shown
      }
      lds_barrier();
      constexpr int PASS = RLO == 0 ? 0 : 1;
      f2_write_blocks(E, tid, emit_map + cl.emit_off + (PASS ? cl.emit_n[0] : 0), cl.emit_n[PASS], s_dst);
    };
    if constexpr (NT <= 6) pass(std::integral_constant<int, 0>{}, std::integral_constant<int, 16 * NT>{});
    else { pass(std::integral_constant<int, 0>{}, std::integral_constant<int, kRowsPassSplit>{}); pass(std::integral_constant<int, kRowsPassSplit>{}, std::integral_constant<int, 16 * NT>{}); }
  }
  };
  static_assert(kRowsClasses == 3, "one instantiation of the batch loop per row class");
  switch (rows_class_of_rows(H + 1)) {
    case 0: run(std::integral_constant<int, kRowsClassNT[0]>{}); break;
    case 1: run(std::integral_constant<int, kRowsClassNT[1]>{}); break;
    default: run(std::integral_constant<int, kRowsClassNT[2]>{}); break;
  }
  const double wsum = wave_sum(cost);
  __syncthreads();
  if (lane == 0) s_red[wv] = wsum;
  __syncthreads();
  if (tid == 0) w.cost_partial[cidx] = (s_red[0] + s_red[1]) + (s_red[2] + s_red[3]);
  if constexpr (TRACE) {
    if (a.trace && lane == 0 && blockIdx.x < 4096) {
      long long* out = a.trace + ((size_t)blockIdx.x * kF2Waves + wv) * 16;
      out[9] = t_entry; out[10] = t_loop0; out[11] = t_loop1; out[12] = (long long)__builtin_amdgcn_s_memtime();
      out[13] = (long long)__builtin_amdgcn_s_getreg((31 << 11) | 4) | ((long long)__builtin_amdgcn_s_getreg((31 << 11) | 20) << 32);
      out[14] = ((long long)nbatch << 8) | rows_class_of_rows(H + 1);
    }
  }
}

void rows_emit_map(int ni, int nc, int flags, std::vector<unsigned>& pass0, std::vector<unsigned>& pass1) {
  pass0.clear(); pass1.clear();
  const int P0 = 6 * ni, H = P0 + rows_cam_rows(flags);
  const bool two = kRowsClassNT[rows_class_of_rows(H + 1)] > 6;
  auto koff = [&](int lc) { return rows_cam_off(flags, lc); };
  auto kcnt = [&](int lc) { return koff(lc + 1) - koff(lc); };
  auto put = [&](int R, int C, int o, int tab_index) {
    const int pass = two && R >= kRowsPassSplit ? 1 : 0;
    (pass ? pass1 : pass0).push_back(rows_emit_entry(f2_tri(R) - (pass ? f2_tri(kRowsPassSplit) : 0) + C, o, tab_index));
  };
  auto put_zero = [&](int R_near, int o, int tab_index) {
    const int pass = two && R_near >= kRowsPassSplit ? 1 : 0;
    (pass ? pass1 : pass0).push_back(rows_emit_entry((int)kRowsEmitZero, o, tab_index));
  };
  for (int la = 0; la < ni; ++la)
    for (int lb = 0; lb <= la; ++lb)
      for (int o = 0; o < 42; ++o) {
        if (o < 36) { const int r = o / 6, c = o % 6; if (la == lb && r < c) continue; put(6 * la + r, 6 * lb + c, o, f2_tri(la) + lb); }
        else if (la == lb) put(H, 6 * la + (o - 36), o, f2_tri(la) + lb);
      }
  for (int lc = 0; lc < nc; ++lc)
    for (int la = 0; la < ni; ++la)
      for (int o = 0; o < 54; ++o) {
        const int r = o / 6;
        if (r < kcnt(lc)) put(P0 + koff(lc) + r, 6 * la + o % 6, o, kF2TabIP + lc * 16 + la);
        else put_zero(P0 + koff(lc), o, kF2TabIP + lc * 16 + la);
      }
  for (int lc = 0; lc < nc; ++lc)
    for (int lc2 = 0; lc2 <= lc; ++lc2)
      for (int o = 0; o < 90; ++o) {
        const int t = kF2TabII + f2_tri(lc) + lc2;
        if (o < 81) {
          const int r = o / 9, c = o % 9;
          if (lc == lc2 && r < c) continue;
          if (r < kcnt(lc) && c < kcnt(lc2)) put(P0 + koff(lc) + r, P0 + koff(lc2) + c, o, t);
          else put_zero(P0 + koff(lc), o, t);
        } else if (lc == lc2) {
          if (o - 81 < kcnt(lc)) put(H, P0 + koff(lc) + (o - 81), o, t);
          else put_zero(H, o, t);
        }
      }
}

void launch_schur_rows(hipStream_t st, const FrontArgs& a, int kmax_intr, bool generic, int num_clusters,
                       const SchurRowsCluster* clusters, const int* tab, const int* cl_lists, const unsigned short* obs_meta,
                       const unsigned long long* lanemap, const unsigned* emit_map, double* part_pp, double* part_ip, double* part_ii,
                       const CamSweepArgs* with_sweep) {
  if (num_clusters <= 0) return;
  RowsSweep sweep{};
  sweep.first = num_clusters;
  if (with_sweep) sweep.cs = *with_sweep;
  static const char* trace_file = std::getenv("MAVBA_ROWS_TRACE");
  static int trace_calls = 0;
  if (trace_file && !with_sweep && !generic && kmax_intr > 4 && kmax_intr <= 8 && ++trace_calls == 5) {
    const size_t trace_n = (size_t)4096 * kF2Waves * 16;
    long long* tr = nullptr;
    (void)hipMalloc(reinterpret_cast<void**>(&tr), trace_n * 8);
    (void)hipMemsetAsync(tr, 0, trace_n * 8, st);
    FrontArgs b = a;
    b.trace = tr;
    hipLaunchKernelGGL((k_schur_rows<8, false, true>), dim3(num_clusters), dim3(kF2Threads), 0, st, b, clusters, tab, cl_lists, obs_meta, lanemap, emit_map, part_pp, part_ip, part_ii, sweep);
    std::vector<long long> hst(trace_n);
    (void)hipStreamSynchronize(st);
    (void)hipMemcpy(hst.data(), tr, trace_n * 8, hipMemcpyDeviceToHost);
    (void)hipFree(tr);
    if (FILE* fp = std::fopen(trace_file, "w")) {
      for (int g = 0; g < std::min(num_clusters, 4096); ++g)
        for (int wv = 0; wv < kF2Waves; ++wv) {
          const long long* rr = hst.data() + ((size_t)g * kF2Waves + wv) * 16;
          if (rr[12] <= 0) continue;
          std::fprintf(fp, "%d %d", g, wv);
          for (int t = 0; t < 15; ++t) std::fprintf(fp, " %lld", rr[t]);
          std::fprintf(fp, "\n");
        }
      std::fclose(fp);
    }
    return;
  }
  const int grid = num_clusters + (with_sweep ? with_sweep->num_chunks : 0);
  with_width_or_none(kmax_intr, [&](auto k) {
    constexpr int K = decltype(k)::value;
    constexpr bool in_place = K == 4 || K == 8;
    with_bool(generic || !in_place, [&](auto g) {
      with_bool(with_sweep != nullptr, [&](auto sw) {
        if constexpr (decltype(g)::value || in_place)
          hipLaunchKernelGGL((k_schur_rows<K, decltype(g)::value, false, decltype(sw)::value>), dim3(grid), dim3(kF2Threads), 0, st, a, clusters, tab,
                             cl_lists, obs_meta, lanemap, emit_map, part_pp, part_ip, part_ii, sweep);
      });
    });
  });
}

}
```

mavmap_amd/csrc/session.h:

```cpp
#ifndef MAVBA_SESSION_H_
#define MAVBA_SESSION_H_
#include <algorithm>
#include <chrono>
#include <cmath>
#include <cstdio>
#include <cstdlib>
#include <cstring>
#include <condition_variable>
#include <functional>
#include <limits>
#include <map>
#include <memory>
#include <mutex>
#include <shared_mutex>
#include <stdexcept>
#include <string>
#include <thread>
#include <unordered_map>
#include <vector>

#include "../../include/mavba.h"
#include "../../include/mavba_triangulate.h"
#include "../../include/mavba_backsub_tiles.h"
#include "../../include/mavba_absolute_pose.h"
#include "../../include/mavba_relative_pose.h"
#include "ba_math.h"
#include "internal.h"

namespace mavba {

extern thread_local std::string g_last_error;

struct Failure : std::runtime_error {
  int code;
  Failure(int c, const std::string& m) : std::runtime_error(m), code(c) {}
};
#define HIP_OK(expr)                                                                     \
  do {                                                                                   \
    hipError_t e_ = (expr);                                                              \
    if (e_ != hipSuccess)                                                                \
      throw Failure(e_ == hipErrorOutOfMemory ? MAVBA_ERR_OUT_OF_MEMORY : MAVBA_ERR_HIP, \
                    std::string(#expr) + ": " + hipGetErrorString(e_));                  \
  } while (0)

template <typename T>
struct DevBuf {
  T* p = nullptr;
  size_t n = 0;
  DevBuf() {}
  DevBuf(const DevBuf&) = delete;
  DevBuf& operator=(const DevBuf&) = delete;
  ~DevBuf() { if (p) device_free(p); }
  void alloc(size_t count) {
    if (p) { device_free(p); p = nullptr; }
    n = count;
    if (count) HIP_OK(device_alloc(reinterpret_cast<void**>(&p), count * sizeof(T)));
  }
  void upload(const std::vector<T>& h, hipStream_t st) {
    alloc(std::max<size_t>(h.size(), 1));
    if (!h.empty()) HIP_OK(copy_h2d_staged(p, h.data(), h.size() * sizeof(T), st));
  }
  void upload(const T* h, size_t count, hipStream_t st) {
    alloc(std::max<size_t>(count, 1));
    if (count) HIP_OK(copy_h2d_staged(p, h, count * sizeof(T), st));
  }
  void upload_pinned(const T* h, size_t count, hipStream_t st) {
    alloc(std::max<size_t>(count, 1));
    if (count) HIP_OK(hipMemcpyAsync(p, h, count * sizeof(T), hipMemcpyHostToDevice, st));
  }
  void zero(hipStream_t st) { if (n) HIP_OK(zero_async(p, n * sizeof(T), st)); }
};

struct ElimNode { std::vector<int> imgs; int parent; };
std::vector<ElimNode> elimination_tree(int NI, int NC, const std::vector<std::vector<int>>& lower, int forced, int max_depth);

struct DeviceRaw { const double* uv; const int* img; const int* pt; const double* points; };
long long device_scan_scratch(long long n);
void device_scan_exclusive(hipStream_t st, unsigned* data, long long n, unsigned* scratch);

struct RcclGuard;
int session_borrow_rccl(mavba_session* s, void* comm, const std::shared_ptr<RcclGuard>& guard, int rank, int world_size);
bool inproc_comms_acquire(int world, const std::vector<int>& device, std::vector<void*>& out, std::shared_ptr<RcclGuard>& guard,
                          std::string& error);
void inproc_comms_abort();
int multi_gpu_ranks();
int solve_multi_gpu(const mavba_problem* P, const mavba_options* options, mavba_result* result, double* point_error, int world);

void pose_refine_batch(int count, mavba_pose_refine_item* items, const mavba_options& opt, mavba_result* results);

void triangulate_pairs(int count, mavba_tri_pair* items, int device);

void absolute_pose_ransac(int count, mavba_abspose_item* items, int device);

void relative_pose_ransac(int count, mavba_relpose_item* items, int device);

void rccl_unique_id(void* out128);
void* rccl_comm_create(const void* id128, int rank, int world);
void rccl_comm_destroy(void* comm);
void rccl_comm_abort(void* comm);
void rccl_allreduce(void* comm, double* p, long long count, int op, hipStream_t stream);
int rccl_comm_async_error(void* comm);
struct RcclGuard {
  std::shared_mutex m;
  bool aborted = false;
};
hipError_t pinned_alloc(void** out, size_t bytes);
// ... 86 lines not shown
      int within = 0;
      for (int t = 0; t < T; ++t) { const int c = hist[t][k]; hist[t][k] = within; within += c; }
      start[k] = within;
      sum += within;
    }
    range_sum[r + 1] = sum;
  });
  for (int r = 0; r < T; ++r) range_sum[r + 1] += range_sum[r];
  run([&](int r) {
    int pos = (int)range_sum[r];
    for (long long k = (long long)nkeys * r / T; k < (long long)nkeys * (r + 1) / T; ++k) {
      const int tot = start[k];
      start[k] = pos;
      for (int t = 0; t < T; ++t) hist[t][k] += pos;
      pos += tot;
    }
  });
  start[nkeys] = (int)range_sum[T];
  run([&](int t) {
    for (long long i = n * t / T; i < n * (t + 1) / T; ++i) emit(i, hist[t][key(i)]++);
  });
}

static inline int model_k(int m) { return m == MAVBA_MODEL_PINHOLE ? 4 : m == MAVBA_MODEL_OPENCV ? 8 : 9; }
static inline int round_up(int x, int m) { return (x + m - 1) / m * m; }
static inline double now_s() {
  return std::chrono::duration<double>(std::chrono::steady_clock::now().time_since_epoch()).count();
}

struct KernelTimer { std::string name; long long launches = 0; double total_ms = 0.0; };

template <typename F>
static void parallel_ranges(long long n, F&& body, long long min_parallel = 200000) {
  int T = (int)std::min<long long>(host_threads(), std::max<long long>(n, 1));
  if (n < min_parallel) T = 1;
  if (T == 1) { body(0ll, n); return; }
  host_run(T, [&](int t) { body(n * t / T, n * (t + 1) / T); });
}

}

using namespace mavba;

struct mavba_session {
  mavba_options opt;
  int device = 0;
  hipStream_t st = nullptr;
  int NI = 0, NC = 0, NP = 0, N = 0, Nstride = 32, NPs = 32, KMAX = 4, n_full = 0, n_pad = 64, Q = 0;
  long long NO_all = 0;
  bool any_intr_free = false;
  std::vector<double> h_poses0, h_intr0, h_points0;
  std::vector<int> h_cam_model, h_img_cam, h_pt_start, h_oimg;
  std::vector<long long> perm;
  std::vector<int> h_pt_count_all;
  std::vector<double> h_dropped_rnorm;
  std::vector<double> h_dropped_cost;
  double fixed_cost_priors = 0.0;
  int num_priors_all = 0;
  std::vector<unsigned char> h_pt_removed;
  DevBuf<unsigned char> d_pt_active;
  std::vector<int> h_pt_orig;
  std::vector<unsigned char> h_pose_const, h_intr_const_in, h_pt_const_in;
  std::vector<unsigned char> h_img_used, h_cam_used, h_pt_used;
  std::vector<unsigned char> h_prior_on_img;
  std::vector<unsigned char> h_pose_free, h_intr_free, h_pt_free;
  double fixed_cost = 0.0;
  long long num_residuals = 0, num_residuals_reduced = 0, num_parameters_reduced = 0;
  int num_priors = 0;
  double prior_weight = 0.0;
  double setup_seconds = 0.0, solve_seconds = 0.0;

  DevBuf<double2> d_uv, d_im_uv;
  DevBuf<int> d_obs_img, d_obs_pt, d_pt_start, d_im_pt, d_img_cam, d_cam_model, d_img_chunk_start,
      d_cam_img_start, d_cam_imgs, d_prior_img, d_prior_start, d_q_pt, d_q_cam, d_q_start, d_pt_count;
  DevBuf<FrontTile> d_front_tiles;
  int num_front_tiles = 0;
  DevBuf<FrontTile> d_tail_tiles;
  int num_tail_tiles = 0, tail_begin = 0;
  bool front_ok = false;
  bool fused_ok = false;
  int eval_rows = 0;
  bool front_valid = false;
  double front_radius = 0.0;
  bool fail_slot_clean = false;
  bool planes_ready = false;
  DevBuf<BsTile> d_bs_tiles;
  int num_bs_tiles = 0;
  int backsub_blocks = -1;
  void read_backsub_switch();
  bool backsub_on_tiles() const { return backsub_blocks < 0 ? !small_window() : backsub_blocks == 0; }
  int backsub_rows() const { return backsub_on_tiles() ? backsub_tiles_grid(num_bs_tiles) : backsub_points_grid(NP); }
  DevBuf<SweepChunk> d_sweep_chunks;
  int num_sweep_chunks = 0;
  DevBuf<unsigned char> d_pose_free, d_intr_free, d_pt_free;
  DevBuf<double> d_prior_R0;
  DevBuf<SchurBlock> d_blocks;
  DevBuf<SchurChunk> d_chunks[3];
  DevBuf<SchurCluster> d_clusters;
  DevBuf<SchurRowsCluster> d_rows_clusters;
  DevBuf<int> d_rows_lists;
  DevBuf<unsigned> d_rows_emit;
  DevBuf<unsigned long long> d_rows_lanes;
  int rows_class_count[kRowsClasses] = {};
  bool rows_ok = false;
  bool rows_generic = false;
  DevBuf<PartialReduce> d_reduce_tasks;
  int num_reduce_tasks = 0;
  DevBuf<int> d_cl_tab, d_cl_lists;
  DevBuf<unsigned short> d_obs_meta, d_q_meta;
  DevBuf<unsigned char> d_pt_clustered;
  int num_clusters = 0, num_slots[3] = {0, 0, 0};
  long long clustered_points = 0, cluster_partials = 0;
  double cluster_flops = 0.0;
  DevBuf<int2> d_terms[3];
  int num_blocks = 0, num_chunks[3] = {0, 0, 0};
  long long num_terms[3] = {0, 0, 0};
  DevBuf<double> d_poses, d_intr, d_points, d_cposes, d_cintr, d_cpoints, d_poses0, d_intr0, d_points0;
  DevBuf<double> d_camrec, d_ccamrec;
  bool camrec_current = false;
  DevBuf<double> d_R, d_Jp, d_Jc, d_Jk, d_Cu, d_gu, d_Gi, d_h, d_scale_cam, d_scale_pt;
  DevBuf<double> d_sweep_partial, d_camsum , d_img_intr_tmp, d_cam_partial;
  DevBuf<double> d_prior_res, d_prior_jac, d_prior_cost;
  DevBuf<double> d_Epose, d_Eintr, d_Wk, d_part[3];
  DevBuf<double> d_M, d_L, d_y, d_diag_ws, d_delta_cam, d_delta_pts, d_norm_partial, d_step_partial, d_scal;
  DevBuf<double> d_rnorm, d_perr;
  DevBuf<int> d_pt_orig;
  DevBuf<int> d_perm32;
  DevBuf<double> d_pts_out;
  double* d_img_rec = nullptr;
  double* d_cam_rec = nullptr;
  CholStructure chol_struct;
  bool prereduced = false;
  bool sweep_rode_along = false;
  bool setup_batched = false;
  bool M_is_clean = false;
  bool allow_persistent = true;
  bool persist_decided = false;
  bool speculate_on = true;
  void decide_persistent();
  int n_mat = 64, nd_parts = 0;
  std::vector<int> h_off_img, h_off_cam, h_col_var;
  DevBuf<int> d_off, d_col_var;
  DevBuf<double> d_ymat;
  DevBuf<int> d_ar_tiles;
  DevBuf<double> d_ar_buf;
  int num_ar_tiles = 0;

  bool evaluated = false, scales_ready = false, started = false, assembled = false;
  double radius = 1e4, decrease_factor = 2.0;
  double cost = 0.0, x_norm = 0.0, grad_max = 0.0, abs_gtol = 0.0, initial_cost = 0.0;
  int iteration = 0, invalid_steps = 0, n_success = 0, n_fail = 0;
  int termination = MAVBA_TERM_RUNNING;

  mavba_allreduce_fn ar_fn = nullptr;
  void* ar_ctx = nullptr;
  void* rccl_comm = nullptr;
  bool rccl_comm_owned = true;
  std::shared_ptr<RcclGuard> rccl_guard;
  bool sharded() const { return (ar_fn || rccl_comm) && (world > 1 || force_exchange); }
  bool force_exchange = false;
  int rank = 0, world = 1;

  std::vector<KernelTimer> timers;
  struct Pending { int idx; hipEvent_t a, b; bool own_a = true; };
  std::vector<Pending> pending;
  std::vector<hipEvent_t> ev_pool;
// ... 16 lines not shown
  hipEvent_t get_event() {
    if (!ev_pool.empty()) { hipEvent_t e = ev_pool.back(); ev_pool.pop_back(); return e; }
    hipEvent_t e; HIP_OK(hipEventCreate(&e)); return e;
  }
  template <typename F>
  void timed(const char* name, F&& f) {
    if (!opt.profile_kernels) { f(); return; }
    Pending p; p.idx = timer_index(name); p.a = get_event(); p.b = get_event();
    HIP_OK(hipEventRecord(p.a, st));
    f();
    HIP_OK(hipEventRecord(p.b, st));
    pending.push_back(p);
  }
  template <typename F>
  void timed_split(const char* first, const char* second, F&& f) {
    if (!opt.profile_kernels) { f(nullptr); return; }
    Pending p, q;
    p.idx = timer_index(first); q.idx = timer_index(second);
    p.a = get_event(); p.b = get_event(); q.a = p.b; q.b = get_event(); q.own_a = false;
    HIP_OK(hipEventRecord(p.a, st));
    f(p.b);
    HIP_OK(hipEventRecord(q.b, st));
    pending.push_back(p); pending.push_back(q);
  }
  void flush_timers() {
    for (auto& p : pending) {
      float ms = 0.f;
      if (hipEventElapsedTime(&ms, p.a, p.b) == hipSuccess) { timers[p.idx].launches++; timers[p.idx].total_ms += ms; }
      if (p.own_a) ev_pool.push_back(p.a);
      ev_pool.push_back(p.b);
    }
    pending.clear();
  }
  void sync() { HIP_OK(hipStreamSynchronize(st)); HIP_OK(hipGetLastError()); release_staged(st); flush_timers(); }
  void download(void* dst, const void* src, size_t bytes) { HIP_OK(copy_d2h_staged_sync(dst, src, bytes, st)); release_staged(st); }

  void allreduce(double* dptr, long long count, int op) {
    if (!sharded()) return;
    if (rccl_comm) {
      if (rccl_guard) {
        std::shared_lock<std::shared_mutex> lk(rccl_guard->m);
        if (rccl_guard->aborted) throw Failure(MAVBA_ERR_HIP, "the communicator group was aborted (another rank failed)");
        rccl_allreduce(rccl_comm, dptr, count, op, st);
      } else {
        rccl_allreduce(rccl_comm, dptr, count, op, st);
      }
      return;
    }
    sync();
    if (ar_fn(ar_ctx, dptr, count, op) != 0) throw Failure(MAVBA_ERR_HIP, "all-reduce hook failed");
  }

  SweepArgs sweep_args(const double* camrec, const double* intr, const double* points) {
    SweepArgs a;
    a.N = N; a.Nstride = Nstride; a.NI = NI; a.NC = NC; a.KMAX = KMAX;
    a.uv = d_uv.p; a.obs_img = d_obs_img.p; a.obs_pt = d_obs_pt.p;
    a.camrec = camrec; a.intr = intr; a.img_cam = d_img_cam.p; a.cam_model = d_cam_model.p;
    a.points = points;
    a.pt_active = h_pt_removed.empty() ? nullptr : d_pt_active.p;
    a.loss_b = opt.loss_scale_factor * opt.loss_scale_factor; a.loss_inv_b = 1.0 / a.loss_b;
    a.R = d_R.p; a.Jp = d_Jp.p; a.Jc = d_Jc.p; a.Jk = d_Jk.p; a.cost_partial = d_sweep_partial.p;
    return a;
  }
  void read_scalars(double* h) {
    HIP_OK(hipMemcpyAsync(h, d_scal.p, SC_COUNT * sizeof(double), hipMemcpyDeviceToHost, st));
    sync();
  }

  void build(const mavba_problem* P, const DeviceRaw* raw = nullptr);
void intr_entries_on_device(const std::vector<unsigned char>& cam_active, std::vector<int>& q_start, std::vector<int>& q_cam);
    void order_on_device(const mavba_problem* P, std::vector<int>& img_start, const DeviceRaw* raw);
  void order_on_host(const mavba_problem* P, const long long* keptp, std::vector<int>& img_start,
                     std::unique_ptr<PinnedBuf<double2>>& uv_h, std::unique_ptr<PinnedBuf<int>>& opt_h,
                     std::unique_ptr<PinnedBuf<double2>>& im_uv_h, std::unique_ptr<PinnedBuf<int>>& im_pt_h);
  void ensure_perm_host();
  void derive_free_flags();
  void finish_structure();
  void choose_elimination_order(const std::vector<SchurBlock>& blocks);
  void reset_state();
  void evaluate(double next_radius = -1.0);
  void evaluate_enqueue(double next_radius = -1.0, const LmSpec& spec = lm_spec_off());
  EvalTailArgs eval_tail_args(const LmSpec& spec);
  CamUpdateArgs cam_update_args(double r);
  void launch_front(double r, bool entries, const LmSpec& spec = lm_spec_off(), const CamSweepArgs* with_sweep = nullptr);
  DevBuf<double> d_lm_dec;
  double* lm_pub = nullptr;
  double lm_seq = 0.0;
  LmSpec lm_spec(bool pending_eval) const {
    LmSpec sp{};
    sp.dec = nullptr; sp.scal = d_scal.p;
    sp.radius = radius; sp.decrease_factor = decrease_factor;
    sp.ptol = opt.parameter_tolerance; sp.ftol = opt.function_tolerance; sp.min_rel_dec = opt.min_relative_decrease;
    sp.max_radius = opt.max_trust_region_radius; sp.abs_gtol = abs_gtol; sp.pending_eval = pending_eval ? 1 : 0;
    return sp;
  }
  bool wait_publication(double* h);
  void build_front_tiles(const std::vector<int>& q_start);
  void build_tiles(const std::vector<int>& q_start, int first, DevBuf<FrontTile>& out, int& count);
  void ensure_planes();
  bool fused_now() const { return fused_ok && rows_ok; }
  int eval_cost_rows() const { return front_ok ? eval_rows : (N > 0 ? jacobian_sweep_grid(N) : 0); }
  void take_evaluation(const double* h) { cost = h[SC_COST]; grad_max = h[SC_GRAD_MAX]; x_norm = std::sqrt(h[SC_XNORM2]); }
  void assemble(double r);
  void solve_linear(double r);
  void linear_step(double r, double* h_scal);
  void candidate(double r, double* h_scal);
  void candidate_enqueue(double r, ReduceTasks* tail = nullptr, int* tail_count = nullptr);
  bool merge_small() const;
  bool small_window() const;
  bool merge_on = true;
  long long sweep_ride_max_obs = -1;
  double pub_wait_seconds = 0.0;
  bool cameras_updated = false;
  double cameras_updated_r = 0.0;
  void start();
  int iterate(int max_iters, int* done);
  void point_errors(double* out);
  void restart();
  long long filter_points(double max_error, const unsigned char* keep, unsigned char* removed_out, double* errors_out);
  void restore_initial_params() {
    HIP_OK(hipMemcpyAsync(d_poses.p, d_poses0.p, (size_t)NI * 6 * 8, hipMemcpyDeviceToDevice, st));
    HIP_OK(hipMemcpyAsync(d_intr.p, d_intr0.p, (size_t)NC * 9 * 8, hipMemcpyDeviceToDevice, st));
    HIP_OK(hipMemcpyAsync(d_points.p, d_points0.p, (size_t)NP * 3 * 8, hipMemcpyDeviceToDevice, st));
    camrec_current = false; evaluated = false; front_valid = false;
  }
  void apply_filter_state();
  void to_caller_points(const double* internal, double* out, int width) const {
    for (int q = 0; q < NP; ++q)
      for (int e = 0; e < width; ++e) out[(size_t)h_pt_orig[q] * width + e] = internal[(size_t)q * width + e];
  }
  void fill_result(mavba_result* r);
};
#endif
```

mavmap_amd/csrc/session_lm.hip:

```cpp
#include "session.h"
#include "lm_decide.h"
#if defined(__x86_64__) || defined(__i386__)
#include <immintrin.h>
#define MAVBA_CPU_RELAX() _mm_pause()
#else
#include <thread>
#define MAVBA_CPU_RELAX() std::this_thread::yield()
#endif

using namespace mavba;


void mavba_session::ensure_planes() {
  if (planes_ready) return;
  d_R.alloc((size_t)2 * Nstride); d_Jp.alloc((size_t)6 * Nstride); d_Jc.alloc((size_t)12 * Nstride);
  d_Jk.alloc((size_t)2 * KMAX * Nstride);
  d_Wk.alloc((size_t)std::max(Q, 1) * 27);
  planes_ready = true;
}

void mavba_session::launch_front(double r, bool entries, const LmSpec& spec, const CamSweepArgs* with_sweep) {
  sweep_rode_along = false;
  prereduced = false;
  FrontArgs f;
  f.spec = spec;
  f.sw = sweep_args(d_camrec.p, d_intr.p, d_points.p);
  f.num_tiles = num_front_tiles; f.NPs = NPs; f.tiles = d_front_tiles.p;
  f.pt_start = d_pt_start.p; f.q_start = d_q_start.p; f.q_cam = d_q_cam.p; f.q_pt = d_q_pt.p;
  f.pt_free = d_pt_free.p; f.scale_cam = d_scale_cam.p; f.scale_pt = d_scale_pt.p;
  f.radius = r; f.dmin = opt.min_lm_diagonal; f.dmax = opt.max_lm_diagonal;
  f.Cu = d_Cu.p; f.gu = d_gu.p; f.Gi = d_Gi.p; f.h = d_h.p; f.Epose = d_Epose.p; f.Eintr = d_Eintr.p;
  f.fail = d_scal.p + SC_FAIL_FRONT;
  f.trace = nullptr;
  static_assert(SC_FAIL_FRONT == SC_FAIL + 1, "the two failure slots are cleared together");
  if (entries) { if (!spec.dec) HIP_OK(hipMemsetAsync(d_scal.p + SC_FAIL, 0, 2 * sizeof(double), st)); fail_slot_clean = true; }
  if (entries && fused_now()) {
    const bool forms_agree = (Q == 0 && !any_intr_free) || (Q > 0 && any_intr_free);
    const CamSweepArgs* ride = (with_sweep && forms_agree) ? with_sweep : nullptr;
    timed("schur_fused", [&] {
      launch_schur_rows(st, f, Q > 0 ? KMAX : 0, rows_generic, num_clusters, d_rows_clusters.p, d_cl_tab.p, d_rows_lists.p, d_obs_meta.p,
                        d_rows_lanes.p, d_rows_emit.p, d_part[0].p, d_part[1].p, d_part[2].p, ride);
    });
    sweep_rode_along = ride != nullptr;
    eval_rows = num_clusters;
    if (num_tail_tiles > 0) {
      FrontArgs t = f;
      t.tiles = d_tail_tiles.p; t.num_tiles = num_tail_tiles;
      t.sw.cost_partial = f.sw.cost_partial + num_clusters;
      timed("point_front", [&] { launch_point_front(st, t, Q > 0 ? KMAX : 0, true); });
      eval_rows += point_front_grid(num_tail_tiles);
    }
  } else {
    timed(entries ? "point_front" : "point_front_sums", [&] { launch_point_front(st, f, Q > 0 ? KMAX : 0, entries); });
    eval_rows = point_front_grid(num_front_tiles);
  }
  front_valid = entries;
  front_radius = r;
}

EvalTailArgs mavba_session::eval_tail_args(const LmSpec& spec) {
  EvalTailArgs e;
  e.NI = NI; e.NC = NC; e.NP = NP; e.NPs = NPs; e.with_cams = any_intr_free ? 1 : 0; e.cam_part = rank == 0 ? 1 : 0;
  state_norms_grid(NI, NC, NP, &e.gp, &e.gc);
  e.img_chunk_start = d_img_chunk_start.p; e.cam_partial = d_cam_partial.p;
  e.prior_start = num_priors > 0 ? d_prior_start.p : nullptr; e.prior_res = d_prior_res.p; e.prior_jac = d_prior_jac.p;
  e.cam_img_start = d_cam_img_start.p; e.cam_imgs = d_cam_imgs.p; e.img_rec = d_img_rec; e.cam_rec = d_cam_rec;
  e.img_intr_tmp = d_img_intr_tmp.p;
  e.pose_free = d_pose_free.p; e.intr_free = d_intr_free.p; e.pt_free = d_pt_free.p;
  e.poses = d_poses.p; e.intr = d_intr.p; e.points = d_points.p; e.gu = d_gu.p; e.norm_partial = d_norm_partial.p;
  const int rows = e.gp + e.gc;
  e.T.t[0] = ReduceTask{d_norm_partial.p, rows, 2, 1, nullptr, 0, d_scal.p + SC_GRAD_MAX};
  e.T.t[1] = ReduceTask{d_norm_partial.p + 1, rows, 2, 0, nullptr, 0, d_scal.p + SC_XNORM2};
  e.T.t[2] = ReduceTask{d_sweep_partial.p, eval_cost_rows(), 1, 0, d_prior_cost.p, num_priors, d_scal.p + SC_COST};
  e.num_tasks = 3;
  e.spec = spec;
  return e;
}

CamUpdateArgs mavba_session::cam_update_args(double r) {
  CamUpdateArgs u;
  u.NI = NI; u.NC = NC; u.cam_part = rank == 0 ? 1 : 0; u.radius = r; u.dmin = opt.min_lm_diagonal; u.dmax = opt.max_lm_diagonal;
  u.scale_cam = d_scale_cam.p; u.img_rec = d_img_rec; u.cam_rec = d_cam_rec; u.poses = d_poses.p; u.intr = d_intr.p;
  u.cand_poses = d_cposes.p; u.cand_intr = d_cintr.p; u.delta_cam = d_delta_cam.p;
  u.partial3 = d_step_partial.p + 3 * (size_t)backsub_rows(); u.cand_camrec = d_ccamrec.p;
  return u;
}

void mavba_session::evaluate_enqueue(double next_radius, const LmSpec& spec) {
  if (!camrec_current) timed("cam_prepare", [&] { launch_cam_prepare(st, NI, d_poses.p, d_camrec.p); });
  camrec_current = true;
  SweepArgs a = sweep_args(d_camrec.p, d_intr.p, d_points.p);
  CamSweepArgs c;
  c.NI = NI; c.NC = NC; c.chunks = d_sweep_chunks.p; c.num_chunks = num_sweep_chunks;
  c.im_uv = d_im_uv.p; c.im_pt = d_im_pt.p; c.camrec = d_camrec.p; c.intr = d_intr.p;
  c.img_cam = d_img_cam.p; c.cam_model = d_cam_model.p; c.points = d_points.p;
  c.pt_active = a.pt_active;
  c.loss_b = a.loss_b; c.loss_inv_b = a.loss_inv_b; c.partial = d_cam_partial.p;
  c.spec = spec;
  sweep_rode_along = false;
  if (front_ok) {
    constexpr long long kProfiledRideMaxObs = 1000000;
    const bool size_ok = (sweep_ride_max_obs < 0 || N <= sweep_ride_max_obs) && !(opt.profile_kernels && N > kProfiledRideMaxObs);
    const bool ride = scales_ready && num_sweep_chunks > 0 && (merge_small() || (merge_on && !sharded() && size_ok));
    launch_front(next_radius, scales_ready && next_radius > 0.0, spec, ride ? &c : nullptr);
  } else {
    ensure_planes();
    front_valid = false;
    timed("jacobian_sweep", [&] { launch_jacobian_sweep(st, a); });
    timed("point_reduce", [&] {
      launch_point_reduce(st, NP, NPs, Nstride, KMAX, d_pt_start.p, d_q_start.p, d_q_cam.p, d_obs_img.p, d_img_cam.p,
                          d_R.p, d_Jp.p, d_Jk.p, d_Cu.p, d_gu.p, d_Wk.p);
    });
  }
  if (!sweep_rode_along) timed("camera_sweep", [&] { launch_camera_sweep(st, c, KMAX, any_intr_free); });
  PartialRide pride;
  static const bool pride_on = [] { const char* e = std::getenv("MAVBA_PARTIAL_RIDE"); return !e || std::atoi(e) != 0; }();
  if (pride_on && merge_on && front_ok && front_valid && fused_now() && num_reduce_tasks > 0 && num_chunks[0] + num_chunks[1] + num_chunks[2] == 0 &&
      num_tail_tiles == 0 && !sharded() && !opt.profile_kernels) {
    pride.n = num_reduce_tasks; pride.tasks = d_reduce_tasks.p; pride.pp = d_part[0].p; pride.ip = d_part[1].p; pride.ii = d_part[2].p;
  }
  if (num_priors > 0)
    timed("rot_prior", [&] {
      launch_rot_prior(st, num_priors, d_prior_img.p, d_prior_R0.p, prior_weight, d_poses.p, d_prior_res.p,
                       d_prior_jac.p, d_prior_cost.p, spec);
    });
  EvalTailArgs e = eval_tail_args(spec);
  if (scales_ready && merge_small()) {
    timed("eval_small", [&] { launch_eval_small(st, e); });
    evaluated = true; assembled = false;
    return;
  }
  e.ride = pride;
  prereduced = pride.n > 0;
  if (scales_ready && merge_on && !sharded() && NI <= 160) {
    timed("eval_tail", [&] { launch_eval_head_tail(st, e); });
    evaluated = true; assembled = false;
    return;
  }
  timed("camera_reduce", [&] { launch_camera_reduce(st, e); });
  allreduce(d_camsum.p, (long long)NI * kImgRec + (long long)NC * kCamRec, 0);
  if (!scales_ready) {
    timed("scales", [&] {
      launch_scales(st, NI, NC, NP, NPs, opt.jacobi_scaling, d_pose_free.p, d_intr_free.p, d_pt_free.p, d_img_rec,
                    d_cam_rec, d_Cu.p, d_scale_cam.p, d_scale_pt.p);
    });
    scales_ready = true;
  }
  timed("state_norms", [&] { launch_state_norms(st, e); });
  timed("reduce", [&] { launch_reduce_tasks(st, e.T, e.num_tasks, spec); });
  if (sharded()) allreduce(d_scal.p + SC_COST, SC_EVAL_COUNT, 2);
  evaluated = true; assembled = false;
}
void mavba_session::evaluate(double next_radius) {
  evaluate_enqueue(next_radius);
  double h[SC_COUNT];
  read_scalars(h);
  take_evaluation(h);
}

void mavba_session::assemble(double r) {
  const double dmin = opt.min_lm_diagonal, dmax = opt.max_lm_diagonal;
  if (front_ok) {
    if (!(front_valid && front_radius == r)) launch_front(r, true);
    else if (!fail_slot_clean) HIP_OK(hipMemsetAsync(d_scal.p + SC_FAIL, 0, sizeof(double), st));
  } else {
    HIP_OK(hipMemsetAsync(d_scal.p + SC_FAIL, 0, sizeof(double), st));
    HIP_OK(hipMemsetAsync(d_scal.p + SC_FAIL_FRONT, 0, sizeof(double), st));
    timed("entries_pose", [&] {
      launch_factor_entries_pose(st, N, Nstride, NPs, d_obs_img.p, d_obs_pt.p, d_pt_free.p, d_Jc.p, d_Jp.p, d_scale_cam.p,
                                 d_scale_pt.p, d_Gi.p, d_h.p, d_Epose.p, d_pt_start.p, d_Cu.p, d_gu.p, r, dmin, dmax,
                                 d_scal.p + SC_FAIL);
    });
    timed("entries_intr", [&] {
      launch_entries_intr(st, Q, NI, NPs, d_q_pt.p, d_q_cam.p, d_Wk.p, d_scale_cam.p, d_scale_pt.p, d_Gi.p, d_h.p,
                          d_Eintr.p);
    });
  }
  if (!M_is_clean) {
    timed("memset_S", [&] {
      HIP_OK(hipMemsetAsync(d_M.p, 0, chol_struct.store_doubles() * sizeof(double), st));
      launch_fix_diag(st, n_mat, chol_struct.d_tile_slot, rank == 0, d_col_var.p, d_scale_cam.p, d_M.p);
    });
    M_is_clean = true;
  }
  if (!(front_ok && fused_now())) timed("schur_clusters", [&] {
    launch_schur_clusters(st, num_clusters, d_clusters.p, d_cl_tab.p, d_pt_start.p, d_q_start.p, d_obs_meta.p,
                          d_q_meta.p, d_pt_clustered.p, d_Epose.p, d_Eintr.p, d_h.p, NPs, d_part[0].p, d_part[1].p,
                          d_part[2].p);
  });
  if (num_chunks[0] > 0) timed("schur_chunks_pp", [&] { launch_schur_chunks(st, BLK_PP, num_chunks[0], d_chunks[0].p, d_terms[0].p, d_Epose.p, d_Eintr.p, d_part[0].p); });
  if (num_chunks[1] > 0) timed("schur_chunks_ip", [&] { launch_schur_chunks(st, BLK_IP, num_chunks[1], d_chunks[1].p, d_terms[1].p, d_Epose.p, d_Eintr.p, d_part[1].p); });
  if (num_chunks[2] > 0) timed("schur_chunks_ii", [&] { launch_schur_chunks(st, BLK_II, num_chunks[2], d_chunks[2].p, d_terms[2].p, d_Epose.p, d_Eintr.p, d_part[2].p); });
  const int nbt = n_mat / 64;
  timed("schur_finalize", [&] {
    if (!(prereduced && front_valid && front_radius == r)) launch_partial_reduce(st, num_reduce_tasks, d_reduce_tasks.p, d_part[0].p, d_part[1].p, d_part[2].p);
    launch_schur_finalize(st, num_blocks, d_blocks.p, d_part[0].p, d_part[1].p, d_part[2].p, NI, NC, chol_struct.d_tile_slot, nbt, rank == 0,
                          r, dmin, dmax, d_img_cam.p, d_img_rec, d_cam_rec, d_scale_cam.p, d_off.p, d_off.p + NI, d_M.p);
  });
  if (sharded()) {
    launch_tiles_copy(st, num_ar_tiles, d_ar_tiles.p, chol_struct.d_tile_slot, nbt, d_M.p, d_ar_buf.p, true);
    allreduce(d_ar_buf.p, (long long)num_ar_tiles * 4096 + n_mat, 0);
    launch_tiles_copy(st, num_ar_tiles, d_ar_tiles.p, chol_struct.d_tile_slot, nbt, d_M.p, d_ar_buf.p, false);
  }
  assembled = true;
}

void mavba_session::decide_persistent() {
  if (persist_decided) return;
  if (chol_struct.persist_ok && !sharded()) allow_persistent = persistent_allowed_now();
  persist_decided = true;
}

void mavba_session::solve_linear(double r) {
  decide_persistent();
  assemble(r);
  const CamUpdateArgs u = cam_update_args(r);
  const bool with_update = merge_small();
  timed_split("chol_factor", "chol_backsolve", [&](hipEvent_t mid) {
    cameras_updated = dense_spd_solve_device(st, d_M.p, n_mat, d_ymat.p, d_scal.p + SC_FAIL, d_diag_ws.p, d_L.p, chol_struct, d_col_var.p, d_y.p,
                                             allow_persistent, mid, with_update ? &u : nullptr);
    cameras_updated_r = r;
  });
  assembled = false;
  fail_slot_clean = false;
  if (!(allow_persistent && chol_struct.persist_ok) || sharded()) M_is_clean = false;
}

void mavba_session::read_backsub_switch() {
  const char* e = std::getenv("MAVBA_BACKSUB_BLOCKS");
  backsub_blocks = e ? (std::atoi(e) != 0 ? 1 : 0) : -1;
}

void mavba_session::linear_step(double r, double* h) {
  read_backsub_switch();
  solve_linear(r);
  candidate(r, h);
  if (h[SC_FAIL] >= 1e29 && allow_persistent) {
    std::fprintf(stderr, "mavba: persistent factorisation timed out, falling back to the launch-per-panel schedule\n");
    allow_persistent = false;
    persistent_timed_out();
    solve_linear(r);
    candidate(r, h);
  }
}

void mavba_session::candidate(double r, double* h) {
  candidate_enqueue(r);
  read_scalars(h);
}
void mavba_session::candidate_enqueue(double r, ReduceTasks* tail, int* tail_count) {
  const double dmin = opt.min_lm_diagonal, dmax = opt.max_lm_diagonal;
  const bool tiles = backsub_on_tiles();
  const int rows = backsub_rows(), ugroups = update_cameras_groups(NI);
  if (!(cameras_updated && cameras_updated_r == r))
    timed("update_cameras", [&] { launch_update_cameras(st, cam_update_args(r), d_y.p); });
  cameras_updated = false;
  static const long long fuse_env = [] { const char* e = std::getenv("MAVBA_COST_FUSE_MAX_OBS"); return e ? std::atoll(e) : -1ll; }();
  const long long fuse_max_obs = fuse_env >= 0 ? fuse_env : 500000ll;
  const bool cost_separate = tiles && fuse_env < 0 ? false : (long long)N > fuse_max_obs;
  double* cost_rows = cost_separate ? nullptr : d_sweep_partial.p;
  timed("backsub_points", [&] {
    if (tiles)
      launch_backsub_points_tiles(st, num_bs_tiles, d_bs_tiles.p, NPs, NI, r, dmin, dmax, sweep_args(d_camrec.p, d_intr.p, d_points.p),
                                  d_pt_start.p, d_delta_cam.p, d_pt_free.p, d_Gi.p, d_h.p, d_Cu.p, d_gu.p, d_scale_pt.p, d_cpoints.p,
                                  d_delta_pts.p, d_step_partial.p, d_ccamrec.p, d_cintr.p, cost_rows);
    else
      launch_backsub_points_jvp(st, NP, NPs, NI, r, dmin, dmax, sweep_args(d_camrec.p, d_intr.p, d_points.p), d_pt_start.p,
                                d_delta_cam.p, d_pt_free.p, d_Gi.p, d_h.p, d_Cu.p, d_gu.p, d_scale_pt.p, d_cpoints.p,
                                d_delta_pts.p, d_step_partial.p, d_ccamrec.p, d_cintr.p, cost_rows);
  });
  SweepArgs a = sweep_args(d_ccamrec.p, d_cintr.p, d_cpoints.p);
  if (cost_separate) timed("cost_only", [&] { launch_cost_only(st, a); });
  if (num_priors > 0)
    timed("rot_prior", [&] {
      launch_rot_prior(st, num_priors, d_prior_img.p, d_prior_R0.p, prior_weight, d_cposes.p, d_prior_res.p,
                       d_prior_jac.p, d_prior_cost.p);
    });
  {
    const int nsweep = N > 0 ? (cost_separate ? jacobian_sweep_grid(N) : rows) : 0;
    ReduceTasks T;
    T.t[0] = ReduceTask{d_step_partial.p, rows + ugroups, 3, 0, nullptr, 0, d_scal.p + SC_STEP_NORM2};
    T.t[1] = ReduceTask{d_step_partial.p + 1, rows + ugroups, 3, 0, nullptr, 0, d_scal.p + SC_MODEL_CHANGE};
    T.t[2] = ReduceTask{d_step_partial.p + 2, rows + ugroups, 3, 0, nullptr, 0, d_scal.p + SC_CAND_XNORM2};
    T.t[3] = ReduceTask{d_sweep_partial.p, nsweep, 1, 0, d_prior_cost.p, num_priors, d_scal.p + SC_NEW_COST};
    if (tail) { *tail = T; *tail_count = 4; }
    else timed("reduce", [&] { launch_reduce_tasks(st, T, 4); });
  }
  if (sharded()) allreduce(d_scal.p + SC_CAND_BEGIN, SC_CAND_COUNT, 0);
}

bool mavba_session::small_window() const {
  return !sharded() && NI <= 64 && NC <= 8 && NP <= 8192 && dense_spd_solve_is_small(n_mat, chol_struct);
}
bool mavba_session::merge_small() const { return merge_on && small_window(); }

void mavba_session::start() {
  { const char* e = std::getenv("MAVBA_MERGE"); merge_on = !e || std::atoi(e) != 0; }
  { const char* e = std::getenv("MAVBA_SPECULATE"); speculate_on = !e || std::atoi(e) != 0; }
  read_backsub_switch();
  { const char* e = std::getenv("MAVBA_SWEEP_RIDE_MAX_OBS"); sweep_ride_max_obs = e ? std::max(0ll, std::atoll(e)) : -1; }
  decide_persistent();
  evaluate();
  initial_cost = cost + fixed_cost;
  const double g0 = std::max(grad_max, std::numeric_limits<double>::epsilon());
  abs_gtol = opt.gradient_tolerance * g0;
  started = true;
  if (num_residuals_reduced == 0 || num_parameters_reduced == 0) { termination = MAVBA_TERM_FUNCTION_TOLERANCE; return; }
  if (grad_max <= abs_gtol) { termination = MAVBA_TERM_GRADIENT_TOLERANCE; return; }
  if (opt.print_progress) {
    std::printf("%4s %14s %12s %10s %10s %10s %10s\n", "iter", "cost", "cost_change", "|gradient|", "|step|", "tr_ratio", "tr_radius");
    std::printf("%4d %14.6e %12.2e %10.2e %10.2e %10.2e %10.2e\n", 0, cost + fixed_cost, 0.0, grad_max, 0.0, 0.0, radius);
  }
}

bool mavba_session::wait_publication(double* h) {
  volatile double* pub = lm_pub;
  const double t_end = now_s() + 2.0;
  for (long long spin = 0;; ++spin) {
    if (pub[SC_COUNT + 7] == lm_seq) break;
    MAVBA_CPU_RELAX();
    if ((spin & 0xFFFF) == 0xFFFF && now_s() > t_end) return false;
  }
  std::atomic_thread_fence(std::memory_order_acquire);
  for (int i = 0; i < SC_COUNT; ++i) h[i] = pub[i];
  return true;
}

int mavba_session::iterate(int max_iters, int* done) {
  const double t0 = now_s();
  int n = 0;
  if (!started) start();
  const bool defer = (!sharded() || rccl_comm || std::getenv("MAVBA_DEFER_WITH_HOOK") != nullptr) && !opt.print_progress;
  const bool speculate = speculate_on && defer && !sharded() && front_ok && fused_now() && rows_ok && scales_ready;
  if (speculate && !lm_pub) { lm_pub = lm_pub_alloc(); if (lm_pub) lm_pub[SC_COUNT + 7] = -1.0; }
  if (speculate && lm_pub && !d_lm_dec.p) d_lm_dec.alloc(2);
  const bool merge_tail = merge_on;
  bool pending_eval = false;
  while (termination == MAVBA_TERM_RUNNING && n < max_iters) {
    if (iteration >= opt.max_num_iterations) { termination = MAVBA_TERM_NO_CONVERGENCE; break; }
    ++iteration; ++n;
    double h[SC_COUNT];
    const LmSpec sp = lm_spec(pending_eval);
    bool speculated = false;
    struct Books { bool evaluated, assembled, front_valid, fail_slot_clean; double front_radius; int eval_rows; bool prereduced; } books{};
    if (speculate && lm_pub) {
      solve_linear(radius);
      lm_seq += 1.0;
      if (merge_tail) {
        ReduceTasks T; int nt = 0;
        candidate_enqueue(radius, &T, &nt);
        timed("lm_tail", [&] { launch_lm_tail(st, T, nt, sp, d_lm_dec.p, lm_pub, lm_seq, d_scal.p + SC_FAIL); });
      } else {
        candidate_enqueue(radius);
        timed("lm_snapshot", [&] { launch_lm_snapshot(st, sp, d_lm_dec.p, lm_pub, lm_seq, d_scal.p + SC_FAIL); });
      }
      books = Books{evaluated, assembled, front_valid, fail_slot_clean, front_radius, eval_rows, prereduced};
      std::swap(d_poses.p, d_cposes.p); std::swap(d_intr.p, d_cintr.p); std::swap(d_points.p, d_cpoints.p);
      std::swap(d_camrec.p, d_ccamrec.p);
      LmSpec ks = sp;
      ks.dec = d_lm_dec.p;
      evaluate_enqueue(1.0 , ks);
      speculated = true;
      const double tw = now_s();
      const bool published = wait_publication(h);
      pub_wait_seconds += now_s() - tw;
      if (!published) {
        sync();
        for (int i = 0; i < SC_COUNT; ++i) h[i] = lm_pub[i];
      }
      if (opt.profile_kernels) sync();
      if (h[SC_FAIL] >= 1e29 && allow_persistent) {
        std::swap(d_poses.p, d_cposes.p); std::swap(d_intr.p, d_cintr.p); std::swap(d_points.p, d_cpoints.p);
        std::swap(d_camrec.p, d_ccamrec.p);
        evaluated = books.evaluated; assembled = books.assembled;
        front_valid = false;
        fail_slot_clean = false; front_radius = books.front_radius; eval_rows = books.eval_rows; prereduced = false;
        speculated = false;
        std::fprintf(stderr, "mavba: persistent factorisation timed out, falling back to the launch-per-panel schedule\n");
        allow_persistent = false;
        persistent_timed_out();
        solve_linear(radius);
        candidate(radius, h);
      }
    } else {
      linear_step(radius, h);
    }
    if (pending_eval) take_evaluation(h);
    const LmDecision dec = lm_decide(h, sp);
    auto forget_speculation = [&] {
      if (!speculated) return;
      std::swap(d_poses.p, d_cposes.p); std::swap(d_intr.p, d_cintr.p); std::swap(d_points.p, d_cpoints.p);
      std::swap(d_camrec.p, d_ccamrec.p);
      evaluated = books.evaluated; assembled = books.assembled; front_valid = books.front_valid;
      fail_slot_clean = false;
      front_radius = books.front_radius; eval_rows = books.eval_rows; prereduced = books.prereduced;
      speculated = false;
    };
    if (dec.code == LM_TERM_GTOL) {
      forget_speculation();
      pending_eval = false;
      termination = MAVBA_TERM_GRADIENT_TOLERANCE;
      --iteration; --n;
      break;
    }
    pending_eval = false;
    if (dec.code == LM_INVALID) {
      forget_speculation();
      if (++invalid_steps >= opt.max_num_consecutive_invalid_steps) { termination = MAVBA_TERM_NUMERICAL_FAILURE; ++n_fail; break; }
    } else {
      invalid_steps = 0;
      if (dec.code == LM_TERM_PTOL) { forget_speculation(); termination = MAVBA_TERM_PARAMETER_TOLERANCE; break; }
      if (dec.code == LM_TERM_FTOL) { forget_speculation(); termination = MAVBA_TERM_FUNCTION_TOLERANCE; break; }
    }
    const bool successful = dec.code == LM_ACCEPTED;
    radius = dec.radius;
    decrease_factor = dec.decrease_factor;
    if (successful) {
      ++n_success;
      if (speculated) {
        front_radius = radius;
        pending_eval = true;
      } else {
        std::swap(d_poses.p, d_cposes.p); std::swap(d_intr.p, d_cintr.p); std::swap(d_points.p, d_cpoints.p);
        std::swap(d_camrec.p, d_ccamrec.p);
        if (defer) {
          evaluate_enqueue(radius);
          pending_eval = true;
        } else {
          evaluate(radius);
          if (grad_max <= abs_gtol) termination = MAVBA_TERM_GRADIENT_TOLERANCE;
        }
      }
    } else {
      forget_speculation();
      ++n_fail;
    }
    if (opt.print_progress)
      std::printf("%4d %14.6e %12.2e %10.2e %10.2e %10.2e %10.2e\n", iteration, cost + fixed_cost, successful ? dec.cost_change : 0.0,
                  grad_max, dec.step_norm, dec.rel, radius);
    if (termination == MAVBA_TERM_RUNNING && radius < opt.min_trust_region_radius) termination = MAVBA_TERM_PARAMETER_TOLERANCE;
  }
  if (pending_eval) {
    double h[SC_COUNT];
    read_scalars(h);
    take_evaluation(h);
    if (grad_max <= abs_gtol) termination = MAVBA_TERM_GRADIENT_TOLERANCE;
  }
  if (termination == MAVBA_TERM_RUNNING && iteration >= opt.max_num_iterations) termination = MAVBA_TERM_NO_CONVERGENCE;
  if (done) *done = n;
  solve_seconds += now_s() - t0;
  return MAVBA_OK;
}

void mavba_session::point_errors(double* out) {
  launch_cam_prepare(st, NI, d_poses.p, d_camrec.p);
  SweepArgs a = sweep_args(d_camrec.p, d_intr.p, d_points.p);
  launch_raw_residual_norm(st, a, d_rnorm.p);
  launch_point_errors(st, NP, d_pt_start.p, d_rnorm.p, d_pt_count.p, d_perr.p);
  std::vector<double> h(NP);
  if (NP) download(h.data(), d_perr.p, (size_t)NP * 8);
  sync();
  evaluated = false;
  for (int p = 0; p < NP; ++p)
    if (h_pt_count_all[p] > 0 && (h_pt_removed.empty() || !h_pt_removed[p])) {
      const int po = h_pt_orig[p];
      out[po] = h_dropped_rnorm.empty() ? h[p] : h[p] + h_dropped_rnorm[po] / (double)h_pt_count_all[p];
    }
}

void mavba_session::restart() {
  evaluated = scales_ready = started = assembled = false;
  front_valid = false;
  cameras_updated = false;
  M_is_clean = false;
  radius = opt.initial_trust_region_radius; decrease_factor = 2.0;
  cost = x_norm = grad_max = abs_gtol = initial_cost = 0.0;
  iteration = invalid_steps = n_success = n_fail = 0;
  termination = MAVBA_TERM_RUNNING;
// ... 80 lines not shown
```

Baseline: 1335 iter/s.

## Fold first-iteration Jacobi scale computation into the Schur front pass

On the first evaluation, before scales exist, the point front now runs in a start mode. It computes point Jacobi scales inline from the row sums, applies them to its own outputs, writes them out, and uses a 0/1 free-table in place of the camera scales. Schur finalize then applies the camera scales afterwards, and the separate scales kernel skips clustered points. This removes one extra front pass at startup, at the cost of another kernel template instantiation and more state to track across speculation rollback. A debug API to read back the scales is also added.

After: 1349 iter/s, median of 6. About the same (+1.1%).

```diff
diff --git a/__graft_entry__.py b/__graft_entry__.py
--- a/__graft_entry__.py
+++ b/__graft_entry__.py
@@ -36,7 +36,7 @@
     import mavmap_amd
     L = mavmap_amd.load()
     from mavmap_amd import api
-    for sym in api.EXPORTED_SYMBOLS + api.TRIANGULATE_SYMBOLS + api.ABSPOSE_SYMBOLS + api.RELPOSE_SYMBOLS + api.BACKSUB_TILES_SYMBOLS:
+    for sym in api.EXPORTED_SYMBOLS + api.TRIANGULATE_SYMBOLS + api.ABSPOSE_SYMBOLS + api.RELPOSE_SYMBOLS + api.BACKSUB_TILES_SYMBOLS + api.DEBUG_SCALES_SYMBOLS:
         getattr(L, sym)
 
 
diff --git a/include/mavba_debug_scales.h b/include/mavba_debug_scales.h
--- /dev/null
+++ b/include/mavba_debug_scales.h
@@ -0,0 +1,15 @@
+#ifndef MAVBA_DEBUG_SCALES_H_
+#define MAVBA_DEBUG_SCALES_H_
+
+#include "mavba.h"
+
+#ifdef __cplusplus
+extern "C" {
+#endif
+
+int mavba_session_debug_scales(mavba_session* s, double* scale_cam, double* scale_pt, double* cu_diag);
+
+#ifdef __cplusplus
+}
+#endif
+#endif
diff --git a/mavmap_amd/api.py b/mavmap_amd/api.py
--- a/mavmap_amd/api.py
+++ b/mavmap_amd/api.py
@@ -28,6 +28,7 @@
 ABSPOSE_SYMBOLS = ["mavba_absolute_pose_ransac"]
 RELPOSE_SYMBOLS = ["mavba_relative_pose_ransac"]
 BACKSUB_TILES_SYMBOLS = ["mavba_debug_backsub_tiles"]
+DEBUG_SCALES_SYMBOLS = ["mavba_session_debug_scales"]
 
 ALLREDUCE_FN = C.CFUNCTYPE(C.c_int, C.c_void_p, C.c_void_p, C.c_int64, C.c_int32)
 
@@ -70,6 +71,7 @@
     L.mavba_session_set_allreduce.argtypes = [sp, ALLREDUCE_FN, C.c_void_p, C.c_int32, C.c_int32]
     L.mavba_session_eval_jacobian.argtypes = [sp, dp, dp, dp, dp, dp]
     L.mavba_session_reduced_dim.argtypes = [sp]
+    L.mavba_session_debug_scales.argtypes = [sp, dp, dp, dp]
     L.mavba_session_reduced_system.argtypes = [sp, C.c_double, dp, dp]
     L.mavba_session_linear_step.argtypes = [sp, C.c_double, dp, dp, dp, dp]
     L.mavba_session_time_jacobian.argtypes = [sp, C.c_int32, C.POINTER(C.c_float)]
@@ -703,6 +705,12 @@
         _check(load().mavba_session_linear_step(self._h, float(radius), _d(dp), _d(di), _d(dx), C.byref(mcc)))
         return dict(d_poses=dp, d_intr=di, d_points=dx, model_cost_change=mcc.value)
 
+    def debug_scales(self):
+        n = load().mavba_session_reduced_dim(self._h)
+        sc, sp, cu = np.zeros(n), np.zeros((3, self.problem.num_points)), np.zeros((3, self.problem.num_points))
+        _check(load().mavba_session_debug_scales(self._h, _d(sc), _d(sp), _d(cu)))
+        return sc, sp, cu
+
     def set_profiling(self, on):
         _check(load().mavba_session_set_profiling(self._h, 1 if on else 0))
 
diff --git a/mavmap_amd/build.py b/mavmap_amd/build.py
--- a/mavmap_amd/build.py
+++ b/mavmap_amd/build.py
@@ -11,7 +11,8 @@
 SOURCES = ["kernels.hip", "schur_rows.hip", "dense_chol.hip", "pose_refine.hip", "triangulate.hip", "absolute_pose.hip", "relative_pose.hip", "host_util.hip", "session_build.hip", "session_lm.hip", "scene.hip", "multi_gpu.hip", "device_setup.hip", "api.hip"]
 HEADERS = ["ba_math.h", "tri_math.h", "p3p_math.h", "e5_math.h", "dev_reduce.h", "internal.h", "session.h", "lm_decide.h", "lm_bodies.h", "sweep_body.h", "launch_dispatch.h", os.path.join("..", "..", "include", "mavba.h"),
            os.path.join("..", "..", "include", "mavba_triangulate.h"), os.path.join("..", "..", "include", "mavba_absolute_pose.h"),
-           os.path.join("..", "..", "include", "mavba_relative_pose.h"), os.path.join("..", "..", "include", "mavba_backsub_tiles.h")]
+           os.path.join("..", "..", "include", "mavba_relative_pose.h"), os.path.join("..", "..", "include", "mavba_backsub_tiles.h"),
+           os.path.join("..", "..", "include", "mavba_debug_scales.h")]
 FLAGS = ["--offload-arch=gfx950", "-O3", "-std=c++17", "-fPIC", "-ffp-contract=on", "-Wall",
          "-Wno-unused-result"]
 FILE_FLAGS = {"dense_chol.hip": ["-mllvm", "-amdgpu-mfma-vgpr-form=1"]}
diff --git a/mavmap_amd/csrc/api.hip b/mavmap_amd/csrc/api.hip
--- a/mavmap_amd/csrc/api.hip
+++ b/mavmap_amd/csrc/api.hip
@@ -408,6 +408,21 @@
   s->sync();
   if (d_points) s->to_caller_points(hdp.data(), d_points, 3);
   if (h[SC_FAIL] != 0.0 || h[SC_FAIL_FRONT] != 0.0) throw Failure(MAVBA_ERR_INVALID_ARGUMENT, "linear solve failed (matrix not positive definite)");
+  return MAVBA_OK;
+  MAVBA_CATCH
+}
+
+int mavba_session_debug_scales(mavba_session* s, double* scale_cam, double* scale_pt, double* cu_diag) {
+  MAVBA_SESSION_TRY(s)
+  if (!s->evaluated || !s->scales_ready) s->evaluate();
+  if (scale_cam && s->n_full) s->download(scale_cam, s->d_scale_cam.p, (size_t)s->n_full * 8);
+  if (scale_pt)
+    for (int k = 0; k < 3 && s->NP; ++k) s->download(scale_pt + (size_t)k * s->NP, s->d_scale_pt.p + (size_t)k * s->NPs, (size_t)s->NP * 8);
+  if (cu_diag) {
+    const int d[3] = {0, 3, 5};
+    for (int k = 0; k < 3 && s->NP; ++k) s->download(cu_diag + (size_t)k * s->NP, s->d_Cu.p + (size_t)d[k] * s->NPs, (size_t)s->NP * 8);
+  }
+  s->sync();
   return MAVBA_OK;
   MAVBA_CATCH
 }
diff --git a/mavmap_amd/csrc/internal.h b/mavmap_amd/csrc/internal.h
--- a/mavmap_amd/csrc/internal.h
+++ b/mavmap_amd/csrc/internal.h
@@ -152,6 +152,8 @@
   double* fail;
   long long* trace;
   LmSpec spec;
+  int start = 0;
+  double* scale_pt_out = nullptr;
 };
 int point_front_grid(int num_tiles);
 void launch_point_front(hipStream_t st, const FrontArgs& a, int kmax_intr, bool entries);
@@ -172,7 +174,9 @@
 void launch_scales(hipStream_t st, int NI, int NC, int NP, int NPs, int jacobi,
                    const unsigned char* pose_free, const unsigned char* intr_free,
                    const unsigned char* pt_free, const double* img_rec, const double* cam_rec,
-                   const double* Cu, double* scale_cam, double* scale_pt);
+                   const double* Cu, double* scale_cam, double* scale_pt,
+                   const unsigned char* pt_skip = nullptr );
+void launch_free_table(hipStream_t st, int NI, int NC, const unsigned char* pose_free, const unsigned char* intr_free, double* table);
 
 constexpr int kStateNormsCamBlocks = 64;
 
@@ -207,7 +211,7 @@
                            int NI, int NC, const int* slot, int nb, bool add_base, double radius, double dmin,
                            double dmax, const int* img_cam, const double* img_rec,
                            const double* cam_rec, const double* scale_cam, const int* off_img, const int* off_cam,
-                           double* S);
+                           double* S, bool start_mode = false );
 void launch_tiles_copy(hipStream_t st, int num_tiles, const int* tiles, const int* slot, int nb, double* M, double* buf, bool to_buf);
 void launch_fix_diag(hipStream_t st, int n_mat, const int* slot, bool add_one, const int* col_var,
                      const double* scale_cam, double* S);
diff --git a/mavmap_amd/csrc/kernels.hip b/mavmap_amd/csrc/kernels.hip
--- a/mavmap_amd/csrc/kernels.hip
+++ b/mavmap_amd/csrc/kernels.hip
@@ -736,7 +736,8 @@
                          const unsigned char* __restrict__ intr_free,
                          const unsigned char* __restrict__ pt_free, const double* __restrict__ img_rec,
                          const double* __restrict__ cam_rec, const double* __restrict__ Cu,
-                         double* __restrict__ scale_cam, double* __restrict__ scale_pt) {
+                         double* __restrict__ scale_cam, double* __restrict__ scale_pt,
+                         const unsigned char* __restrict__ pt_skip) {
   const int t = blockIdx.x * blockDim.x + threadIdx.x;
   const int ncam = 6 * NI + 9 * NC;
   if (t < ncam) {
@@ -752,7 +753,7 @@
     }
     scale_cam[t] = fr ? (jacobi ? 1.0 / (1.0 + sqrt(n2)) : 1.0) : 0.0;
   }
-  if (t < NP) {
+  if (t < NP && !(pt_skip && pt_skip[t])) {
     const bool fr = pt_free[t] != 0;
     const int d[3] = {0, 3, 5};
 #pragma unroll
@@ -763,11 +764,22 @@
 void launch_scales(hipStream_t st, int NI, int NC, int NP, int NPs, int jacobi,
                    const unsigned char* pose_free, const unsigned char* intr_free,
                    const unsigned char* pt_free, const double* img_rec, const double* cam_rec,
-                   const double* Cu, double* scale_cam, double* scale_pt) {
+                   const double* Cu, double* scale_cam, double* scale_pt, const unsigned char* pt_skip) {
   const int n = max(6 * NI + 9 * NC, NP);
   if (n <= 0) return;
   hipLaunchKernelGGL(k_scales, dim3((n + 255) / 256), dim3(256), 0, st, NI, NC, NP, NPs, jacobi, pose_free,
-                     intr_free, pt_free, img_rec, cam_rec, Cu, scale_cam, scale_pt);
+                     intr_free, pt_free, img_rec, cam_rec, Cu, scale_cam, scale_pt, pt_skip);
+}
+__global__ void k_free_table(int NI, int NC, const unsigned char* __restrict__ pose_free, const unsigned char* __restrict__ intr_free,
+                             double* __restrict__ table) {
+  const int t = blockIdx.x * blockDim.x + threadIdx.x;
+  if (t < 6 * NI) table[t] = pose_free[t] != 0 ? 1.0 : 0.0;
+  else if (t < 6 * NI + 9 * NC) table[t] = intr_free[t - 6 * NI] != 0 ? 1.0 : 0.0;
+}
+void launch_free_table(hipStream_t st, int NI, int NC, const unsigned char* pose_free, const unsigned char* intr_free, double* table) {
+  const int n = 6 * NI + 9 * NC;
+  if (n <= 0) return;
+  hipLaunchKernelGGL(k_free_table, dim3((n + 255) / 256), dim3(256), 0, st, NI, NC, pose_free, intr_free, table);
 }
 
 __global__ void __launch_bounds__(256) k_state_norms(
@@ -1296,7 +1308,7 @@
     int add_base, double radius, double dmin, double dmax, const int* __restrict__ img_cam,
     const double* __restrict__ img_rec, const double* __restrict__ cam_rec,
     const double* __restrict__ scale_cam, const int* __restrict__ off_img, const int* __restrict__ off_cam,
-    double* __restrict__ S) {
+    double* __restrict__ S, int start_mode) {
   const int wv = threadIdx.x >> 6, lane = threadIdx.x & 63;
   const int bid = blockIdx.x * 4 + wv;
   if (bid >= num_blocks) return;
@@ -1315,6 +1327,7 @@
     if (idx < NA) {
       const int r = idx / RY, c = idx - r * RY;
       const int gr = row0 + r, gc = col0 + c;
+      if (start_mode) s *= scale_cam[gr] * scale_cam[gc];
       double base = 0.0;
       if (add_base) {
         const double sr = scale_cam[gr], sc = scale_cam[gc];
@@ -1340,6 +1353,7 @@
     } else if (is_diag) {
       const int r = idx - NA;
       const int gr = row0 + r;
+      if (start_mode) s *= scale_cam[gr];
       double base = 0.0;
       if (add_base) {
         const double g = B.kind == BLK_PP ? img_rec[(size_t)B.row_ent * kImgRec + 21 + r]
@@ -1357,11 +1371,11 @@
                            int NI, int NC, const int* slot, int nb, bool add_base, double radius, double dmin,
                            double dmax, const int* img_cam, const double* img_rec,
                            const double* cam_rec, const double* scale_cam, const int* off_img, const int* off_cam,
-                           double* S) {
+                           double* S, bool start_mode) {
   if (num_blocks <= 0) return;
   hipLaunchKernelGGL(k_schur_finalize, dim3((num_blocks + 3) / 4), dim3(256), 0, st, num_blocks, blocks, part_pp,
                      part_ip, part_ii, NI, NC, slot, nb, add_base ? 1 : 0, radius, dmin, dmax, img_cam, img_rec, cam_rec,
-                     scale_cam, off_img, off_cam, S);
+                     scale_cam, off_img, off_cam, S, start_mode ? 1 : 0);
 }
 __global__ void __launch_bounds__(256) k_tiles_copy(int num_tiles, const int* __restrict__ tiles, const int* __restrict__ slot, int nb,
                                                     double* __restrict__ M, double* __restrict__ buf, int to_buf) {
diff --git a/mavmap_amd/csrc/schur_rows.hip b/mavmap_amd/csrc/schur_rows.hip
--- a/mavmap_amd/csrc/schur_rows.hip
+++ b/mavmap_amd/csrc/schur_rows.hip
@@ -160,7 +160,7 @@
 }
 
 struct RowsSweep { CamSweepArgs cs; int first; };
-template <int KMAX, bool GENERIC, bool TRACE = false, bool SWEEP = false>
+template <int KMAX, bool GENERIC, bool TRACE = false, bool SWEEP = false, bool START = false>
 __global__ void __launch_bounds__(kF2Threads, 2) k_schur_rows(
     FrontArgs a, const SchurRowsCluster* __restrict__ clusters, const int* __restrict__ tabs, const int* __restrict__ cl_lists,
     const unsigned short* __restrict__ obs_meta, const unsigned long long* __restrict__ lanemap,
@@ -244,8 +244,12 @@
     if (act_n) { im_n = w.obs_img[ob + oi]; m_n = w.uv[ob + oi]; meta_n = obs_meta[ob + oi]; }
     X_n[0] = w.points[3 * (size_t)p]; X_n[1] = w.points[3 * (size_t)p + 1]; X_n[2] = w.points[3 * (size_t)p + 2];
     free_n = a.pt_free[p] != 0;
-#pragma unroll
-    for (int k = 0; k < 3; ++k) sp_n[k] = a.scale_pt[(size_t)k * NPs + p];
+    if constexpr (START) {
+      sp_n[0] = sp_n[1] = sp_n[2] = 1.0;
+    } else {
+#pragma unroll
+      for (int k = 0; k < 3; ++k) sp_n[k] = a.scale_pt[(size_t)k * NPs + p];
+    }
   };
   auto request_batch = [&](int bj) {
     const int pj = bj * kRowsBatch + r;
@@ -267,7 +271,7 @@
     lds_barrier();
     mark();
     constexpr int K3 = KMAX > 0 ? 3 * KMAX : 1;
-    const double sp[3] = {own_free ? own_sp[0] : 0.0, own_free ? own_sp[1] : 0.0, own_free ? own_sp[2] : 0.0};
+    double sp[3] = {own_free ? own_sp[0] : 0.0, own_free ? own_sp[1] : 0.0, own_free ? own_sp[2] : 0.0};
     double jc[12], jps[6], s9[9], P[K3];
 #pragma unroll
     for (int e = 0; e < 9; ++e) s9[e] = 0.0;
@@ -329,6 +333,24 @@
 #if !(MAVBA_ROWS_SKIP & 16)
     row16_allsum(s9);
 #endif
+    if constexpr (START) {
+      if (a.start == 1) {
+        sp[0] = own_free ? 1.0 / (1.0 + sqrt(s9[0])) : 0.0;
+        sp[1] = own_free ? 1.0 / (1.0 + sqrt(s9[3])) : 0.0;
+        sp[2] = own_free ? 1.0 / (1.0 + sqrt(s9[5])) : 0.0;
+        if (act) {
+#pragma unroll
+          for (int e = 0; e < 6; ++e) jps[e] *= sp[e % 3];
+        }
+#pragma unroll
+        for (int u = 0; u < K3; ++u) P[u] *= sp[u % 3];
+      }
+      if (valid && i == 0) {
+        const int p = cl.p0 + pj;
+#pragma unroll
+        for (int k = 0; k < 3; ++k) a.scale_pt_out[(size_t)k * NPs + p] = sp[k];
+      }
+    }
     double G[6] = {0, 0, 0, 0, 0, 0}, hh[3] = {0, 0, 0};
     bool fin = true;
     if (own_free) {
@@ -555,7 +577,7 @@
   if (with_sweep) sweep.cs = *with_sweep;
   static const char* trace_file = std::getenv("MAVBA_ROWS_TRACE");
   static int trace_calls = 0;
-  if (trace_file && !with_sweep && !generic && kmax_intr > 4 && kmax_intr <= 8 && ++trace_calls == 5) {
+  if (trace_file && !with_sweep && a.start == 0 && !generic && kmax_intr > 4 && kmax_intr <= 8 && ++trace_calls == 5) {
     const size_t trace_n = (size_t)4096 * kF2Waves * 16;
     long long* tr = nullptr;
     (void)hipMalloc(reinterpret_cast<void**>(&tr), trace_n * 8);
@@ -586,9 +608,11 @@
     constexpr bool in_place = K == 4 || K == 8;
     with_bool(generic || !in_place, [&](auto g) {
       with_bool(with_sweep != nullptr, [&](auto sw) {
-        if constexpr (decltype(g)::value || in_place)
-          hipLaunchKernelGGL((k_schur_rows<K, decltype(g)::value, false, decltype(sw)::value>), dim3(grid), dim3(kF2Threads), 0, st, a, clusters, tab,
-                             cl_lists, obs_meta, lanemap, emit_map, part_pp, part_ip, part_ii, sweep);
+        with_bool(a.start != 0, [&](auto first) {
+          if constexpr (decltype(g)::value || in_place)
+            hipLaunchKernelGGL((k_schur_rows<K, decltype(g)::value, false, decltype(sw)::value, decltype(first)::value>), dim3(grid), dim3(kF2Threads), 0, st,
+                               a, clusters, tab, cl_lists, obs_meta, lanemap, emit_map, part_pp, part_ip, part_ii, sweep);
+        });
       });
     });
   });
diff --git a/mavmap_amd/csrc/session.h b/mavmap_amd/csrc/session.h
--- a/mavmap_amd/csrc/session.h
+++ b/mavmap_amd/csrc/session.h
@@ -22,6 +22,7 @@
 #include "../../include/mavba.h"
 #include "../../include/mavba_triangulate.h"
 #include "../../include/mavba_backsub_tiles.h"
+#include "../../include/mavba_debug_scales.h"
 #include "../../include/mavba_absolute_pose.h"
 #include "../../include/mavba_relative_pose.h"
 #include "ba_math.h"
@@ -274,6 +275,10 @@
   int eval_rows = 0;
   bool front_valid = false;
   double front_radius = 0.0;
+  bool start_two_pass = false;
+  bool front_start_form = false;
+  DevBuf<double> d_free_table;
+  bool start_one_pass_ok() const;
   bool fail_slot_clean = false;
   bool planes_ready = false;
   DevBuf<BsTile> d_bs_tiles;
@@ -456,7 +461,7 @@
   void evaluate_enqueue(double next_radius = -1.0, const LmSpec& spec = lm_spec_off());
   EvalTailArgs eval_tail_args(const LmSpec& spec);
   CamUpdateArgs cam_update_args(double r);
-  void launch_front(double r, bool entries, const LmSpec& spec = lm_spec_off(), const CamSweepArgs* with_sweep = nullptr);
+  void launch_front(double r, bool entries, const LmSpec& spec = lm_spec_off(), const CamSweepArgs* with_sweep = nullptr, bool start_form = false);
   DevBuf<double> d_lm_dec;
   double* lm_pub = nullptr;
   double lm_seq = 0.0;
diff --git a/mavmap_amd/csrc/session_lm.hip b/mavmap_amd/csrc/session_lm.hip
--- a/mavmap_amd/csrc/session_lm.hip
+++ b/mavmap_amd/csrc/session_lm.hip
@@ -19,7 +19,7 @@
   planes_ready = true;
 }
 
-void mavba_session::launch_front(double r, bool entries, const LmSpec& spec, const CamSweepArgs* with_sweep) {
+void mavba_session::launch_front(double r, bool entries, const LmSpec& spec, const CamSweepArgs* with_sweep, bool start_form) {
   sweep_rode_along = false;
   prereduced = false;
   FrontArgs f;
@@ -32,6 +32,12 @@
   f.Cu = d_Cu.p; f.gu = d_gu.p; f.Gi = d_Gi.p; f.h = d_h.p; f.Epose = d_Epose.p; f.Eintr = d_Eintr.p;
   f.fail = d_scal.p + SC_FAIL_FRONT;
   f.trace = nullptr;
+  if (start_form) {
+    if (!d_free_table.p) d_free_table.alloc((size_t)std::max(6 * NI + 9 * NC, 1));
+    launch_free_table(st, NI, NC, d_pose_free.p, d_intr_free.p, d_free_table.p);
+    f.scale_cam = d_free_table.p; f.scale_pt_out = d_scale_pt.p;
+    f.start = opt.jacobi_scaling ? 1 : 2;
+  }
   static_assert(SC_FAIL_FRONT == SC_FAIL + 1, "the two failure slots are cleared together");
   if (entries) { if (!spec.dec) HIP_OK(hipMemsetAsync(d_scal.p + SC_FAIL, 0, 2 * sizeof(double), st)); fail_slot_clean = true; }
   if (entries && fused_now()) {
@@ -56,6 +62,12 @@
   }
   front_valid = entries;
   front_radius = r;
+  front_start_form = start_form;
+}
+
+bool mavba_session::start_one_pass_ok() const {
+  return !start_two_pass && !opt.profile_kernels && front_ok && fused_now() && num_clusters > 0 && num_tail_tiles == 0 && num_chunks[0] + num_chunks[1] + num_chunks[2] == 0 &&
+         !sharded() && !small_window() && d_pt_clustered.p != nullptr;
 }
 
 EvalTailArgs mavba_session::eval_tail_args(const LmSpec& spec) {
@@ -101,8 +113,11 @@
   if (front_ok) {
     constexpr long long kProfiledRideMaxObs = 1000000;
     const bool size_ok = (sweep_ride_max_obs < 0 || N <= sweep_ride_max_obs) && !(opt.profile_kernels && N > kProfiledRideMaxObs);
-    const bool ride = scales_ready && num_sweep_chunks > 0 && (merge_small() || (merge_on && !sharded() && size_ok));
-    launch_front(next_radius, scales_ready && next_radius > 0.0, spec, ride ? &c : nullptr);
+    if (!scales_ready) { const char* e = std::getenv("MAVBA_START_TWO_PASS"); start_two_pass = e && std::atoi(e) != 0; }
+    const bool start_form = !scales_ready && start_one_pass_ok();
+    const bool ride = (scales_ready || start_form) && num_sweep_chunks > 0 && (merge_small() || (merge_on && !sharded() && size_ok));
+    if (start_form) launch_front(next_radius > 0.0 ? next_radius : radius, true, spec, ride ? &c : nullptr, true);
+    else launch_front(next_radius, scales_ready && next_radius > 0.0, spec, ride ? &c : nullptr);
   } else {
     ensure_planes();
     front_valid = false;
@@ -142,7 +157,7 @@
   if (!scales_ready) {
     timed("scales", [&] {
       launch_scales(st, NI, NC, NP, NPs, opt.jacobi_scaling, d_pose_free.p, d_intr_free.p, d_pt_free.p, d_img_rec,
-                    d_cam_rec, d_Cu.p, d_scale_cam.p, d_scale_pt.p);
+                    d_cam_rec, d_Cu.p, d_scale_cam.p, d_scale_pt.p, front_start_form ? d_pt_clustered.p : nullptr);
     });
     scales_ready = true;
   }
@@ -195,7 +210,8 @@
   timed("schur_finalize", [&] {
     if (!(prereduced && front_valid && front_radius == r)) launch_partial_reduce(st, num_reduce_tasks, d_reduce_tasks.p, d_part[0].p, d_part[1].p, d_part[2].p);
     launch_schur_finalize(st, num_blocks, d_blocks.p, d_part[0].p, d_part[1].p, d_part[2].p, NI, NC, chol_struct.d_tile_slot, nbt, rank == 0,
-                          r, dmin, dmax, d_img_cam.p, d_img_rec, d_cam_rec, d_scale_cam.p, d_off.p, d_off.p + NI, d_M.p);
+                          r, dmin, dmax, d_img_cam.p, d_img_rec, d_cam_rec, d_scale_cam.p, d_off.p, d_off.p + NI, d_M.p,
+                          front_start_form && front_valid && front_radius == r);
   });
   if (sharded()) {
     launch_tiles_copy(st, num_ar_tiles, d_ar_tiles.p, chol_struct.d_tile_slot, nbt, d_M.p, d_ar_buf.p, true);
@@ -342,7 +358,7 @@
     double h[SC_COUNT];
     const LmSpec sp = lm_spec(pending_eval);
     bool speculated = false;
-    struct Books { bool evaluated, assembled, front_valid, fail_slot_clean; double front_radius; int eval_rows; bool prereduced; } books{};
+    struct Books { bool evaluated, assembled, front_valid, fail_slot_clean; double front_radius; int eval_rows; bool prereduced, front_start_form; } books{};
     if (speculate && lm_pub) {
       solve_linear(radius);
       lm_seq += 1.0;
@@ -354,7 +370,7 @@
         candidate_enqueue(radius);
         timed("lm_snapshot", [&] { launch_lm_snapshot(st, sp, d_lm_dec.p, lm_pub, lm_seq, d_scal.p + SC_FAIL); });
       }
-      books = Books{evaluated, assembled, front_valid, fail_slot_clean, front_radius, eval_rows, prereduced};
+      books = Books{evaluated, assembled, front_valid, fail_slot_clean, front_radius, eval_rows, prereduced, front_start_form};
       std::swap(d_poses.p, d_cposes.p); std::swap(d_intr.p, d_cintr.p); std::swap(d_points.p, d_cpoints.p);
       std::swap(d_camrec.p, d_ccamrec.p);
       LmSpec ks = sp;
@@ -374,7 +390,7 @@
         std::swap(d_camrec.p, d_ccamrec.p);
         evaluated = books.evaluated; assembled = books.assembled;
         front_valid = false;
-        fail_slot_clean = false; front_radius = books.front_radius; eval_rows = books.eval_rows; prereduced = false;
+        fail_slot_clean = false; front_radius = books.front_radius; eval_rows = books.eval_rows; prereduced = false; front_start_form = false;
         speculated = false;
         std::fprintf(stderr, "mavba: persistent factorisation timed out, falling back to the launch-per-panel schedule\n");
         allow_persistent = false;
@@ -393,7 +409,7 @@
       std::swap(d_camrec.p, d_ccamrec.p);
       evaluated = books.evaluated; assembled = books.assembled; front_valid = books.front_valid;
       fail_slot_clean = false;
-      front_radius = books.front_radius; eval_rows = books.eval_rows; prereduced = books.prereduced;
+      front_radius = books.front_radius; eval_rows = books.eval_rows; prereduced = books.prereduced; front_start_form = books.front_start_form;
       speculated = false;
     };
     if (dec.code == LM_TERM_GTOL) {
```
